# spthm/grace-devel

Measured on AMD Instinct MI355X. Metric: Mrays/s SPH column-density trace, 10^7 particles, higher is better.
Workload: dtype f32

## Files before the change

grace-devel_amd/csrc/trace.hip:

```cpp
#include "kernel_tables.hpp"
#include "trace_kernel.hpp"
#include "trace_plan.hpp"

#include <cmath>

using namespace grace_hip;

namespace grace_hip {

static_assert(GRACE_SPH_KERNEL_TABLE_ROWS == GRACE_SPH_KERNEL_WENDLAND_C6 + 1, "one table per built-in kernel");
__device__ double g_sph_kernel_tables[GRACE_SPH_KERNEL_TABLE_ROWS][N_TABLE] = GRACE_SPH_KERNEL_TABLES_INIT;
static const double k_sph_kernel_tables[GRACE_SPH_KERNEL_TABLE_ROWS][N_TABLE] = GRACE_SPH_KERNEL_TABLES_INIT;

static grace_status trace_state_destroy(Context& c)
{
    if (!c.trace) return GRACE_OK;
    TraceState& ts = *c.trace;
    GRACE_TRY(plan_release(ts));
    GRACE_TRY(scene_release(ts));
    GRACE_TRY(rays_release(ts));
    if (ts.hits.chunk_counts) GRACE_TRY_HIP(hipFree(ts.hits.chunk_counts));
    if (ts.custom_table) GRACE_TRY_HIP(hipFree(ts.custom_table));
    if (ts.status) GRACE_TRY_HIP(hipFree(ts.status));
    if (ts.ev0) GRACE_TRY_HIP(hipEventDestroy(ts.ev0));
// ... 18 lines not shown
    *out = c->trace;
    return GRACE_OK;
}

}

namespace {

struct LaunchPlan {
    int width = 64, n_packets = 0;
    int split = 1;
    bool dev_split = false;
    int hit_chunk_shift = GRANULE_SHIFT, hit_chunks = 0, hit_split = 1;
    size_t hit_packets = 0;
    bool hits_split = false;
    bool keep_chunks = false;
    bool reorder = false;
    bool lattice = false;
    int lat_split = 0;
    bool fast_b = false;
    int treelet = 0, treelet_axis = 0;
};

template <int MODE>
LaunchPlan plan_launch(const TraceState& ts, const bool keep_requested, const size_t n_rays, const size_t n_prims)
{
    LaunchPlan p;
    while ((((n_prims - 1) >> p.hit_chunk_shift) + 1) > size_t(MAX_HIT_CHUNKS)) ++p.hit_chunk_shift;
    p.hit_chunks = int(((n_prims - 1) >> p.hit_chunk_shift) + 1);
    p.hit_packets = ceil_div(n_rays, size_t(64));
    const bool split_hits = ts.width <= 0 && p.hit_packets < 4096 && p.hit_chunks >= 8 && ts.split != 1;
    p.hits_split = MODE == MODE_HITS && split_hits;
    p.keep_chunks = MODE == MODE_COUNT && keep_requested && split_hits;
    if (p.hits_split) {
        if (ts.split > 0) p.hit_split = ts.split;
        else while (p.hit_split < 8 && p.hit_packets * p.hit_split < 16384) p.hit_split *= 2;
    }
    if (ts.width > 0) p.width = ts.width;
    else if (ordered(MODE) && !p.hits_split)
        while (p.width > 16 && ceil_div(n_rays, size_t(p.width)) < 4096) p.width /= 2;
    else if (class_split(MODE) && ts.split <= 0)
        while (p.width > 16 && ceil_div(n_rays, size_t(p.width)) * SUM_CLASSES < 4096) p.width /= 2;
    p.n_packets = ceil_div(n_rays, size_t(p.width));
    p.reorder = ts.ray_reorder && n_rays > 64;
    if (class_split(MODE)) {
        const size_t wave_budget = f4_sums(MODE) ? 16385 : 16384;
        if (ts.split > 0) p.split = ts.split;
        else {
            while (p.split < SUM_CLASSES && size_t(p.n_packets) * p.split < wave_budget) p.split *= 2;
            if (f4_sums(MODE) && p.split > 1 && p.split < ts.lat_split && p.reorder && p.width == 64)
                p.split = ts.lat_split;
        }
    }
    if (p.hits_split) p.split = p.hit_split;
    p.dev_split = f4_class_split(MODE) && p.split > 1 && ts.split <= 0;
    p.lattice = has_lattice(MODE) && p.reorder;
    if (f4_class_split(MODE) && p.split == 1 && p.lattice && p.width == 64
        && ts.lat_split > 0 && ts.split <= 0)
        p.lat_split = ts.lat_split;
    p.fast_b = f4_sums(MODE) && !ts.exact_integrals;
    const int auto_treelet = (MODE == MODE_TRI) ? 512 : 8192, auto_treelet_axis = 32768;
#ifdef GRACE_PACKET_STATS
    p.treelet = ts.treelet < 0 ? auto_treelet : ts.treelet;
    p.treelet_axis = ts.treelet < 0 ? auto_treelet_axis : ts.treelet;
#else
    p.treelet = (MODE == MODE_STATS) ? 0 : (ts.treelet < 0 ? auto_treelet : ts.treelet);
    p.treelet_axis = (MODE == MODE_STATS) ? 0 : (ts.treelet < 0 ? auto_treelet_axis : ts.treelet);
#endif
    return p;
}

struct Nested { bool on = false; size_t* measure = nullptr; };

struct TraceBuffers {
    unsigned long long* sig = nullptr;
    float4* A = nullptr; float2* B = nullptr; double* T64 = nullptr; int2* node_prims = nullptr; float4* C = nullptr;
    float* partial = nullptr; double* partial_d = nullptr;
    int *chunk_counts = nullptr, *chunk_off = nullptr, *scratch_counts = nullptr;
    int4* wave_map = nullptr; int *n_wave_map = nullptr, *pk_first = nullptr, *pk_parts = nullptr;
    uint32_t *pk_prefix = nullptr, *pk_total = nullptr;
    uint32_t* ext = nullptr; uint32_t* keys = nullptr; uint32_t* perm = nullptr;
    bool plan_eligible = false;
    PlanKey plan_key;
};

template <int MODE>
grace_status use_records(TraceState& ts, TraceArgs& a, TraceBuffers& b, FrameGuard& frame, const LaunchPlan& p,
                         const size_t n_rays, const size_t n_prims, const size_t n_nodes, hipStream_t stream,
                         const Nested nested = Nested())
{
    enum CacheUse { USE_NONE, USE_FILL, USE_CHECK, USE_TRUST };
    auto decide = [&](const bool have, const bool pinned, const bool repeat) {
        if (have) return ts.cache_validation ? USE_CHECK : USE_TRUST;
        return (ts.cache_auto && repeat && !pinned) ? USE_FILL : USE_NONE;
    };
    CacheUse scene_use = USE_NONE, rays_use = USE_NONE;
    const SceneKey skey{primitive(MODE), a.spheres, a.nodes, a.leaves, n_prims, n_nodes};
    if (!fp64(MODE) && MODE != MODE_STATS && !nested.measure) {
        scene_use = decide(ts.scene.valid && ts.scene.key == skey, ts.scene.valid && ts.scene.pinned,
                           ts.scene.seen == skey);
        ts.scene.seen = skey;
        if (scene_use == USE_FILL && scene_cache_alloc(ts, skey) != GRACE_OK) scene_use = USE_NONE;
    }
    const RayKey rkey{a.rays, n_rays};
    if (p.reorder && !nested.on) {
        rays_use = decide(ts.rays.valid && ts.rays.key == rkey, ts.rays.valid && ts.rays.pinned,
                          ts.rays.seen == rkey);
        ts.rays.seen = rkey;
        if (rays_use == USE_FILL && rays_cache_alloc(ts, rkey) != GRACE_OK) rays_use = USE_NONE;
    }
    const bool scene_cached = scene_use != USE_NONE, rays_cached = rays_use != USE_NONE;
    auto held = [](const CacheUse u) { return u == USE_CHECK || u == USE_TRUST; };
    b.plan_eligible = ts.plan_on && f4_sums(MODE) && held(scene_use) && held(rays_use) && p.lat_split == 0;
    if (b.plan_eligible)
        b.plan_key = PlanKey{ PLAN_FORMAT, p.fast_b, group_shift(n_prims), p.width, p.reorder, n_rays, n_prims, ts.scene.gen, ts.rays.gen };
    PlanGate gate;
    const bool plan_steady = b.plan_eligible && ts.plan.valid && ts.plan.key == b.plan_key;
    if (plan_steady) {
        gate.ctl = ts.plan.ctl; gate.scene = ts.scene.ctl; gate.rays = ts.rays.ctl;
    }
    const bool scene_sig = scene_use == USE_FILL || scene_use == USE_CHECK;
    const bool rays_sig = rays_use == USE_FILL || rays_use == USE_CHECK, sig = scene_sig || rays_sig;
    auto carve = [&](char* const base) {
        size_t used = 0;
        auto take = [&](auto*& ptr, const size_t count) {
            using T = std::remove_reference_t<decltype(*ptr)>;
            ptr = base ? reinterpret_cast<T*>(base + used) : nullptr;
            used += Workspace::aligned(count * sizeof(T));
        };
        if (sig) take(b.sig, sig_partial_words());
        if (!scene_cached) {
            take(b.A, n_prims + 4);
            if (f4_integrals(MODE)) take(b.B, n_prims + 4);
            if (MODE == MODE_TRI) take(b.T64, 9 * (n_prims + 4));
            take(b.node_prims, n_nodes); take(b.C, cluster_record_count(n_prims));
        }
        if (f4_sums(MODE)) take(b.partial, n_rays * SUM_CLASSES * channels(MODE));
        if (double_sums(MODE)) take(b.partial_d, n_rays * SUM_CLASSES);
        if (p.hits_split) {
            take(b.chunk_counts, n_rays * size_t(p.hit_chunks)); take(b.chunk_off, n_rays * size_t(p.hit_chunks));
            take(b.scratch_counts, n_rays); take(b.wave_map, p.hit_packets * p.hit_split); take(b.n_wave_map, 16);
            take(b.pk_prefix, p.hit_packets * size_t(p.hit_chunks));
            take(b.pk_total, p.hit_packets + 16); take(b.pk_first, p.hit_packets + 16); take(b.pk_parts, p.hit_packets + 16);
        }
        if (p.reorder) { take(b.ext, 20); take(b.keys, n_rays); take(b.perm, n_rays); }
        return used;
    };
    const size_t own = carve(nullptr);
    const size_t need = own + (p.reorder ? sort_ws_bytes(n_rays, 4, 0) : 0);
    if (nested.measure) {
        *nested.measure = need + Workspace::aligned(sig_partial_words() * sizeof(*b.sig));
        return GRACE_OK;
    }
    if (nested.on) GRACE_REQUIRE(Workspace::room() >= need, "trace: the caller's frame is too small for a nested trace");
    else GRACE_TRY(frame.begin(need, stream));
    carve(Workspace::take<char>(own));
    if (sig) {
        SigRequest rq;
        if (scene_sig) {
            rq.prims = a.spheres; rq.prims_bytes = n_prims * (MODE == MODE_TRI ? 36 : 16);
            rq.nodes = a.nodes; rq.nodes_bytes = n_nodes * 64;
            rq.leaves = a.leaves; rq.leaves_bytes = (n_nodes + 1) * 16;
            rq.scene_ctl = ts.scene.ctl; rq.scene_force = scene_use == USE_FILL;
        }
        if (rays_sig) {
            rq.rays = a.rays; rq.rays_bytes = n_rays * 28;
            rq.rays_ctl = ts.rays.ctl; rq.rays_force = rays_use == USE_FILL; rq.rays_ext = ts.rays.ext;
        }
        GRACE_TRY(launch_signatures(rq, b.sig, stream));
    }
    if (scene_cached) {
        Scene& sc = ts.scene;
        if (scene_use != USE_TRUST) {
            GRACE_TRY(scene_fill(skey.kind, a.spheres, n_prims, a.nodes, n_nodes, a.leaves, sc.A, sc.B1, sc.B50,
                                 sc.T64, sc.node_prims, sc.C, stream, &sc.ctl->stale));
            sc.valid = true;
        }
        a.A = sc.A; a.T64 = sc.T64; a.node_prims = sc.node_prims; a.C = sc.C;
        a.B = f4_integrals(MODE) ? (p.fast_b ? sc.B50 : sc.B1) : nullptr;
    } else {
        GRACE_TRY(scene_fill(skey.kind, primitive(MODE) == PRIM_D4 ? static_cast<const void*>(a.spheres_d) : a.spheres,
                             n_prims, a.nodes, n_nodes, a.leaves, b.A, p.fast_b ? nullptr : b.B, p.fast_b ? b.B : nullptr,
                             b.T64, b.node_prims, b.C, stream));
        a.A = b.A; a.B = b.B; a.T64 = b.T64; a.node_prims = b.node_prims; a.C = b.C;
    }
    if (p.reorder) {
        const float4* scene_min = a.C + 2 * ((n_prims + 63) / 64);
        uint32_t* lat_flag = p.lattice ? b.ext + 13 : nullptr;
        int* split_dev = p.dev_split ? reinterpret_cast<int*>(b.ext + 12) : nullptr;
        const int split_flags = f4_sums(MODE) ? SPLIT_WIDE_BUDGET : 0;
        if (rays_cached) {
            RayOrder& ro = ts.rays;
            if (rays_use != USE_TRUST) {
                GRACE_TRY(ray_order(a.rays, n_rays, ro.ext, b.keys, ro.perm, nullptr, nullptr, 0, 0, nullptr,
                                    stream, &ro.ctl->stale));
                ro.valid = true;
            }
            int* plan_split_dev = b.plan_eligible && split_dev && !weighted(MODE)
                ? reinterpret_cast<int*>(b.ext + 16) : nullptr;
            if (lat_flag || split_dev || plan_steady)
                GRACE_TRY(launch_choose_variants(ro.ext, int(n_rays), scene_min, lat_flag, p.n_packets,
                                                 p.split | split_flags, split_dev, stream, plan_steady ? &gate : nullptr,
                                                 plan_split_dev));
            a.perm = ro.perm; a.plan_split_dev = plan_split_dev;
        } else {
            GRACE_TRY(ray_order(a.rays, n_rays, b.ext, b.keys, b.perm, scene_min, lat_flag, p.n_packets,
                                p.split | split_flags, split_dev, stream));
            a.perm = b.perm;
        }
        a.lat_dev = reinterpret_cast<const int*>(lat_flag); a.split_dev = split_dev;
    }
    return GRACE_OK;
}

template <int MODE, bool SPLIT, bool ALT = false>
void launch_walk(const int grid, const TraceArgs& args, hipStream_t stream)
{
    trace_kernel<MODE, SPLIT, ALT, false><<<grid, TRACE_BLOCK, 0, stream>>>(args);
    if constexpr (has_lattice(MODE))
        if (args.lat_dev) trace_kernel<MODE, SPLIT, ALT, true><<<grid, TRACE_BLOCK, 0, stream>>>(args);
}

template <int MODE>
grace_status dispatch(const TraceState& ts, const TraceArgs& a, const TraceBuffers& b, const LaunchPlan& p,
                      const int* kept, const size_t n_rays, hipStream_t stream)
{
    const int grid = ceil_div(size_t(p.n_packets) * p.split, TRACE_BLOCK / 64);
    const int* const plan_k_dev = a.plan_usable ? a.plan_split_dev : nullptr;
    auto combine = [&](const int k, const int* k_dev, const int* run_if) -> grace_status {
        const int g = ceil_div(n_rays * channels(MODE), 256);
        if constexpr (double_sums(MODE))
            combine_classes_kernel<double><<<g, 256, 0, stream>>>(a.partial_d, int(n_rays), k, k_dev, a.out_sums_d, run_if);
        else if constexpr (weighted(MODE))
            combine_channel_classes_kernel<<<g, 256, 0, stream>>>(a.partial, int(n_rays), channels(MODE), k, k_dev,
                                                                  a.out_sums, a.out_stride, run_if,
                                                                  a.plan_usable, plan_k_dev);
        else if constexpr (f4_sums(MODE))
            combine_classes_kernel<float><<<g, 256, 0, stream>>>(a.partial, int(n_rays), k, k_dev, a.out_sums, run_if,
                                                                 a.plan_usable, plan_k_dev);
        else return GRACE_OK;
        GRACE_CHECK_LAUNCH();
        return GRACE_OK;
    };
    if constexpr (class_split(MODE)) {
        auto walk = [&](auto alt_tag) -> grace_status {
            constexpr bool ALT = decltype(alt_tag)::value;
            if constexpr (has_lattice(MODE)) if (p.lat_split) {
                if (output(MODE) == OUT_COUNTS)
                    GRACE_TRY_HIP(hipMemsetAsync(a.out_counts, 0, n_rays * sizeof(int), stream));
                trace_kernel<MODE, false, ALT, false><<<grid, TRACE_BLOCK, 0, stream>>>(a);
                GRACE_CHECK_LAUNCH();
                TraceArgs a_lat = a;
                a_lat.split = p.lat_split; a_lat.split_dev = nullptr;
                trace_kernel<MODE, true, ALT, true><<<ceil_div(size_t(p.n_packets) * p.lat_split, TRACE_BLOCK / 64),
                                                      TRACE_BLOCK, 0, stream>>>(a_lat);
                GRACE_CHECK_LAUNCH();
                return combine(p.lat_split, nullptr, a.lat_dev);
            }
            if constexpr (f4_sums(MODE)) if (a.plan_usable) {
                GRACE_TRY(plan_record(ts, a, stream));
                const int grid_planned = a.plan_split_dev
                    ? ceil_div(size_t(p.n_packets) * planned_split(p.n_packets), TRACE_BLOCK / 64) : grid;
                GRACE_TRY(launch_planned(MODE, ALT, grid_planned, a, stream));
                if (p.split == 1) GRACE_TRY(combine(1, nullptr, reinterpret_cast<const int*>(a.plan_usable)));
            }
            if (p.split > 1) launch_walk<MODE, true, ALT>(grid, a, stream);
            else launch_walk<MODE, false, ALT>(grid, a, stream);
            return GRACE_OK;
        };
        if constexpr (f4_sums(MODE)) GRACE_TRY(p.fast_b ? walk(std::true_type()) : walk(std::false_type()));
        else GRACE_TRY(walk(std::false_type()));
    } else if constexpr (MODE == MODE_HITS) {
        if (p.hits_split) {
            const int* counts = kept;
            if (!kept) {
                TraceArgs c = a;
                c.chunk_counts = b.chunk_counts; c.out_counts = b.scratch_counts;
                GRACE_TRY_HIP(hipMemsetAsync(b.chunk_counts, 0, n_rays * size_t(p.hit_chunks) * 4, stream));
                GRACE_TRY_HIP(hipMemsetAsync(b.scratch_counts, 0, n_rays * 4, stream));
                launch_walk<MODE_COUNT, true>(grid, c, stream);
                GRACE_CHECK_LAUNCH();
                counts = b.chunk_counts;
            }
            hits_offsets_kernel<<<ceil_div(n_rays, 4), 256, 0, stream>>>(counts, a.offsets, int(n_rays),
                                                                         p.hit_chunks, b.chunk_off);
            GRACE_CHECK_LAUNCH();
            hits_plan_kernel<<<p.n_packets, MAX_HIT_CHUNKS, 0, stream>>>(counts, a.perm, int(n_rays),
                                                                         p.hit_chunks, b.pk_prefix, b.pk_total);
            GRACE_CHECK_LAUNCH();
            hits_assign_kernel<<<1, 1024, 0, stream>>>(b.pk_total, p.n_packets, p.n_packets * p.split, p.hit_chunks,
                                                       b.pk_first, b.pk_parts, b.n_wave_map,
                                                       ts.hits_stage_split ? 200000ull : 0ull);
            GRACE_CHECK_LAUNCH();
            hits_bounds_kernel<<<p.n_packets, 64, 0, stream>>>(b.pk_prefix, b.pk_total, b.pk_first, b.pk_parts,
                                                               p.hit_chunks, b.wave_map);
            GRACE_CHECK_LAUNCH();
            TraceArgs staged = a, direct = a;
            staged.stage_dev = direct.stage_dev = b.n_wave_map + 4;
            staged.stage_want = 1; direct.stage_want = 0;
            launch_walk<MODE, true, true>(grid, staged, stream);
            GRACE_CHECK_LAUNCH();
            launch_walk<MODE, true, false>(grid, direct, stream);
        } else if (p.n_packets >= 4096) {
            launch_walk<MODE, false, true>(grid, a, stream);
        } else {
            launch_walk<MODE, false, false>(grid, a, stream);
        }
    } else {
        launch_walk<MODE, false>(grid, a, stream);
    }
    GRACE_CHECK_LAUNCH();
    GRACE_TRY(stamps_report(MODE));
    if (p.split > 1) GRACE_TRY(combine(p.split, a.split_dev, nullptr));
    return GRACE_OK;
}

template <int MODE>
grace_status launch_trace(TraceArgs a, size_t n_rays, size_t n_spheres, size_t n_nodes,
                          hipStream_t stream, const Nested nested = Nested())
{
    GRACE_REQUIRE(a.rays && a.spheres && a.nodes && a.leaves && a.root, "trace: null pointer");
    GRACE_REQUIRE(n_rays < (size_t(1) << 31), "trace: bad ray count");
    GRACE_REQUIRE(n_nodes >= 1 && n_nodes < (size_t(1) << 30), "trace: bad node count");
    GRACE_REQUIRE(n_spheres > 0 && n_spheres < (size_t(1) << 31), "trace: bad primitive count");
    TraceState* ts_ptr = nullptr;
    GRACE_TRY(trace_state(&ts_ptr));
    TraceState& ts = *ts_ptr;
    GRACE_TRY(ensure_status(ts, stream));
    a.kernel_table = ts.kernel_table;
    const LaunchPlan p = plan_launch<MODE>(ts, a.keep_chunks, n_rays, n_spheres);
    const bool reuse_chunks = p.hits_split && ts.hits.valid && ts.hits.rays == a.rays
        && ts.hits.n_rays == n_rays && ts.hits.prims == static_cast<const void*>(a.spheres)
        && ts.hits.n_prims == n_spheres && ts.hits.n_chunks == p.hit_chunks;
    if (chunked(MODE)) ts.hits.valid = false;
    const size_t need = n_rays * size_t(p.hit_chunks);
    if (p.keep_chunks && ts.hits.capacity < need) {
        if (ts.hits.chunk_counts) { GRACE_TRY_HIP(hipDeviceSynchronize()); GRACE_TRY_HIP(hipFree(ts.hits.chunk_counts)); }
        ts.hits.chunk_counts = nullptr; ts.hits.capacity = 0;
        hipError_t e = hipMalloc(reinterpret_cast<void**>(&ts.hits.chunk_counts), need * sizeof(int));
        if (e != hipSuccess) return set_error(GRACE_OUT_OF_MEMORY, __FILE__, __LINE__, hipGetErrorString(e));
        ts.hits.capacity = need;
    }
    FrameGuard frame;
    TraceBuffers b;
    GRACE_TRY(use_records<MODE>(ts, a, b, frame, p, n_rays, n_spheres, n_nodes, stream, nested));
    if (nested.measure) return GRACE_OK;
    a.width = p.width; a.split = p.split; a.treelet = p.treelet; a.treelet_axis = p.treelet_axis;
    a.n_rays = int(n_rays); a.n_nodes = int(n_nodes); a.n_prims = int(n_spheres); a.status = ts.status;
    a.group_shift = group_shift(n_spheres); a.chunk_shift = p.hit_chunk_shift; a.n_chunks = p.hit_chunks;
    a.partial = b.partial; a.partial_d = b.partial_d;
    a.chunk_off = b.chunk_off; a.wave_map = b.wave_map; a.n_wave_map = b.n_wave_map;
    if (p.split > 1 && output(MODE) == OUT_COUNTS)
        GRACE_TRY_HIP(hipMemsetAsync(a.out_counts, 0, n_rays * sizeof(int), stream));
    if (p.keep_chunks && p.split > 1) {
        a.chunk_counts = ts.hits.chunk_counts;
        GRACE_TRY_HIP(hipMemsetAsync(ts.hits.chunk_counts, 0, n_rays * size_t(p.hit_chunks) * 4, stream));
        ts.hits.valid = true; ts.hits.rays = a.rays; ts.hits.n_rays = n_rays;
        ts.hits.prims = a.spheres; ts.hits.n_prims = n_spheres; ts.hits.n_chunks = p.hit_chunks;
    }
    ts.last_lat_dev = a.lat_dev; ts.last_lat_stream = stream;
    if constexpr (f4_sums(MODE)) {
        PacketPlan& pp = ts.plan;
        if (b.plan_eligible && !(pp.key == b.plan_key && (pp.valid || pp.dead)))
            GRACE_TRY(plan_fill(ts, b.plan_key, a, stream));
        ts.last_plan_ctl = nullptr;
        if (b.plan_eligible && pp.valid && pp.key == b.plan_key) {
            a.plan_idx = pp.idx; a.plan_hdr = pp.hdr; a.plan_spans = pp.spans; a.plan_counts = pp.counts;
            a.plan_usable = &pp.ctl->usable;
            ts.last_plan_ctl = pp.ctl; ts.last_plan_stream = stream;
            ts.last_plan_fuses = !weighted(MODE) && p.fast_b;
        }
    }
    return timed(ts, stream, [&] {
        return dispatch<MODE>(ts, a, b, p, reuse_chunks ? ts.hits.chunk_counts : nullptr, n_rays, stream);
    });
}

TraceArgs trace_args(const void* d_rays, const void* d_prims, const int* d_nodes, const int* d_leaves,
                     const int* d_root)
{
    TraceArgs a = {};
    a.rays = static_cast<const float*>(d_rays);
    a.spheres = static_cast<const float4*>(d_prims);
    a.nodes = reinterpret_cast<const float4*>(d_nodes);
    a.leaves = reinterpret_cast<const int4*>(d_leaves);
    a.root = d_root;
    return a;
}

}

namespace grace_hip {
grace_status rays_invalidate_if_written(const void* d_written)
{
    Context* c = nullptr;
    GRACE_TRY(current_context(&c));
    if (!c->trace) return GRACE_OK;
    TraceState& ts = *c->trace;
    if (ts.cache_validation) return GRACE_OK;
    if (ts.rays.valid && d_written && d_written == static_cast<const void*>(ts.rays.key.rays)) return rays_release(ts);
    return GRACE_OK;
}

grace_status scene_invalidate_if_written(const void* d_written)
{
    Context* c = nullptr;
    GRACE_TRY(current_context(&c));
    if (!c->trace) return GRACE_OK;
    TraceState& ts = *c->trace;
    if (ts.cache_validation) return GRACE_OK;
    if (ts.scene.valid && d_written
        && (d_written == ts.scene.key.prims || d_written == ts.scene.key.nodes || d_written == ts.scene.key.leaves))
        return scene_release(ts);
    return GRACE_OK;
}

grace_status trace_nested_bytes(size_t n_rays, size_t n_spheres, size_t n_nodes, size_t* bytes)
{
    TraceArgs a = trace_args(bytes, bytes, reinterpret_cast<const int*>(bytes), reinterpret_cast<const int*>(bytes),
                             reinterpret_cast<const int*>(bytes));
    size_t counts = 0, hits = 0;
    GRACE_TRY(launch_trace<MODE_COUNT>(a, n_rays, n_spheres, n_nodes, nullptr, Nested{true, &counts}));
    GRACE_TRY(launch_trace<MODE_HITS>(a, n_rays, n_spheres, n_nodes, nullptr, Nested{true, &hits}));
    *bytes = counts > hits ? counts : hits;
    return GRACE_OK;
}

grace_status trace_hitcounts_nested(const void* d_rays, size_t n_rays, const float* d_spheres, size_t n_spheres,
                                    const int* d_nodes, size_t n_nodes, const int* d_leaves, const int* d_root,
                                    int* d_hit_counts, hipStream_t stream)
{
    TraceArgs a = trace_args(d_rays, d_spheres, d_nodes, d_leaves, d_root);
    a.out_counts = d_hit_counts;
    return launch_trace<MODE_COUNT>(a, n_rays, n_spheres, n_nodes, stream, Nested{true, nullptr});
}

grace_status trace_hits_nested(const void* d_rays, size_t n_rays, const float* d_spheres, size_t n_spheres,
                               const int* d_nodes, size_t n_nodes, const int* d_leaves, const int* d_root,
                               const int* d_ray_offsets, int* d_hit_indices, float* d_hit_integrals,
                               float* d_hit_distances, hipStream_t stream)
{
    TraceArgs a = trace_args(d_rays, d_spheres, d_nodes, d_leaves, d_root);
    a.offsets = d_ray_offsets;
    a.hit_idx = d_hit_indices;
    a.hit_integral = d_hit_integrals;
    a.hit_dist = d_hit_distances;
    return launch_trace<MODE_HITS>(a, n_rays, n_spheres, n_nodes, stream, Nested{true, nullptr});
// ... 276 lines not shown
    GRACE_TRACE_STATE();
    GRACE_REQUIRE(ts.timing && ts.ev_valid, "no timed traversal launch recorded");
    GRACE_TRY_HIP(hipEventSynchronize(ts.ev1));
    GRACE_TRY_HIP(hipEventElapsedTime(h_ms, ts.ev0, ts.ev1));
    return GRACE_OK;
}

grace_status grace_trace_last_lattice(int* h_lattice)
{
    GRACE_REQUIRE(h_lattice, "null output");
    *h_lattice = 0;
    GRACE_TRACE_STATE();
    if (ts.last_lat_dev) {
        GRACE_TRY_HIP(hipStreamSynchronize(ts.last_lat_stream));
        GRACE_TRY_HIP(hipMemcpy(h_lattice, ts.last_lat_dev, sizeof(int), hipMemcpyDeviceToHost));
    }
    return GRACE_OK;
}

grace_status grace_trace_last_plan_used(int* h_used)
{
    GRACE_REQUIRE(h_used, "null output");
    *h_used = 0;
    GRACE_TRACE_STATE();
    if (ts.last_plan_ctl) {
        PlanCtl h = {};
        GRACE_TRY_HIP(hipStreamSynchronize(ts.last_plan_stream));
        GRACE_TRY_HIP(hipMemcpy(&h, ts.last_plan_ctl, sizeof(h), hipMemcpyDeviceToHost));
        *h_used = h.usable != 0u ? 1 : 0;
    }
    return GRACE_OK;
}

grace_status grace_trace_plan_stats(unsigned long long* h_stats)
{
    GRACE_REQUIRE(h_stats, "null output");
    for (int k = 0; k < 7; ++k) h_stats[k] = 0;
    GRACE_TRACE_STATE();
    if (ts.last_plan_ctl) {
        PlanCtl h = {};
        GRACE_TRY_HIP(hipStreamSynchronize(ts.last_plan_stream));
        GRACE_TRY_HIP(hipMemcpy(&h, ts.last_plan_ctl, sizeof(h), hipMemcpyDeviceToHost));
        if (h.usable != 0u) {
            for (int k = 0; k < 6; ++k) h_stats[k] = h.stats[k];
            h_stats[6] = h.largest_round;
        }
    }
    return GRACE_OK;
}

grace_status grace_trace_plan_loops(unsigned long long* h_loops)
{
    GRACE_REQUIRE(h_loops, "null output");
    h_loops[0] = h_loops[1] = 0;
    GRACE_TRACE_STATE();
    if (ts.last_plan_ctl) {
        PlanCtl h = {};
        GRACE_TRY_HIP(hipStreamSynchronize(ts.last_plan_stream));
        GRACE_TRY_HIP(hipMemcpy(&h, ts.last_plan_ctl, sizeof(h), hipMemcpyDeviceToHost));
        if (h.usable != 0u) {
            h_loops[0] = ts.last_plan_fuses ? h.loops : h.stats[2];
            h_loops[1] = ts.last_plan_fuses ? h.largest_loop : h.largest_round;
        }
    }
    return GRACE_OK;
}

grace_status grace_trace_set_plan(int on)
{
    GRACE_TRACE_STATE();
    ts.plan_on = on != 0;
    if (!ts.plan_on) GRACE_TRY(plan_release(ts));
    return GRACE_OK;
}

grace_status grace_trace_set_plan_budget(size_t bytes)
{
    GRACE_TRACE_STATE();
    ts.plan_budget = bytes;
    GRACE_TRY(plan_release(ts));
    return GRACE_OK;
}

grace_status grace_trace_plan_bytes(size_t* h_bytes)
{
    GRACE_REQUIRE(h_bytes, "null output");
    GRACE_TRACE_STATE();
    const PacketPlan& pp = ts.plan;
    *h_bytes = pp.valid ? pp.bytes() : 0;
    return GRACE_OK;
}

grace_status grace_trace_set_packet_split(int waves_per_packet)
{
    GRACE_REQUIRE(waves_per_packet == -1 || waves_per_packet == 1 || waves_per_packet == 2
                      || waves_per_packet == 4 || waves_per_packet == 8,
                  "packet split must be 1, 2, 4, 8 or -1 (automatic)");
    GRACE_TRACE_STATE();
    ts.split = waves_per_packet;
    return GRACE_OK;
}

grace_status grace_trace_set_packet_width(int rays_per_packet)
{
    GRACE_REQUIRE(rays_per_packet == -1 || rays_per_packet == 16 || rays_per_packet == 32
                      || rays_per_packet == 64,
                  "packet width must be 16, 32, 64 or -1 (automatic)");
    GRACE_TRACE_STATE();
    ts.width = rays_per_packet;
    return GRACE_OK;
}

grace_status grace_trace_set_exact_integrals(int enabled)
{
    GRACE_TRACE_STATE();
    ts.exact_integrals = enabled != 0;
    return GRACE_OK;
}

grace_status grace_trace_set_sph_kernel(int kind)
{
    GRACE_REQUIRE(kind >= GRACE_SPH_KERNEL_CUBIC && kind <= GRACE_SPH_KERNEL_WENDLAND_C6,
                  "set_sph_kernel: kind must be a built-in GRACE_SPH_KERNEL_* (0..5); a custom table is "
                  "set with grace_trace_set_sph_kernel_table");
    GRACE_TRACE_STATE();
    ts.sph_kernel = kind;
    ts.kernel_table = ts.builtin_tables + kind * N_TABLE;
    return GRACE_OK;
}

grace_status grace_trace_set_sph_kernel_table(const double* h_table, int n)
{
    GRACE_REQUIRE(h_table && n == N_TABLE, "set_sph_kernel_table: the table must hold 51 values");
    for (int i = 0; i < N_TABLE; ++i)
        GRACE_REQUIRE(std::isfinite(h_table[i]) && h_table[i] >= 0.0,
                      "set_sph_kernel_table: every value must be finite and >= 0");
    GRACE_REQUIRE(h_table[N_TABLE - 1] == 0.0, "set_sph_kernel_table: the last value (b = H) must be 0");
    GRACE_TRACE_STATE();
    GRACE_TRY_HIP(hipDeviceSynchronize());
    if (!ts.custom_table)
        GRACE_TRY_HIP(hipMalloc(reinterpret_cast<void**>(&ts.custom_table), N_TABLE * sizeof(double)));
    GRACE_TRY_HIP(hipMemcpy(ts.custom_table, h_table, N_TABLE * sizeof(double), hipMemcpyHostToDevice));
    for (int i = 0; i < N_TABLE; ++i) ts.custom_host[i] = h_table[i];
    ts.sph_kernel = GRACE_SPH_KERNEL_CUSTOM;
    ts.kernel_table = ts.custom_table;
    return GRACE_OK;
}

grace_status grace_trace_get_sph_kernel(int* h_kind, double* h_table51)
{
    GRACE_TRACE_STATE();
    if (h_kind) *h_kind = ts.sph_kernel;
    if (h_table51) {
        const double* t = ts.sph_kernel == GRACE_SPH_KERNEL_CUSTOM ? ts.custom_host
                                                                   : k_sph_kernel_tables[ts.sph_kernel];
        for (int i = 0; i < N_TABLE; ++i) h_table51[i] = t[i];
    }
    return GRACE_OK;
}

grace_status grace_trace_set_treelet_size(int max_primitives)
{
    GRACE_REQUIRE(max_primitives >= -1, "treelet size must be >= 0 (or -1 for automatic)");
    GRACE_TRACE_STATE();
    ts.treelet = max_primitives;
    return GRACE_OK;
// ... 68 lines not shown
```

grace-devel_amd/csrc/trace_coherence.hip:

```cpp
#include "trace_state.hpp"

using namespace grace_hip;

namespace {

__device__ __forceinline__ uint32_t f2ord_u(float f)
{
    const uint32_t u = __float_as_uint(f);
    return (u & 0x80000000u) ? ~u : (u | 0x80000000u);
}

__device__ __forceinline__ float ord2f_u(uint32_t u)
{
    return __uint_as_float((u & 0x80000000u) ? (u & 0x7fffffffu) : ~u);
}

__global__ void ray_ext_init_kernel(uint32_t* __restrict__ ext16)
{
    if (threadIdx.x < 16) ext16[threadIdx.x] = threadIdx.x < 6 ? 0xFFFFFFFFu : 0u;
}

__global__ __launch_bounds__(1024) void ray_extents_kernel(const float* __restrict__ rays, int n,
                                                          uint32_t* __restrict__ ext12,
                                                          const uint32_t* __restrict__ run_if)
// ... 85 lines not shown
    int dims[2] = { 0, 0 }, nvar = 0;
    float lo[2] = { 0.f, 0.f }, span[2] = { 0.f, 0.f };
    for (int k = 5; k >= 0; --k) {
        const float l = ord2f_u(ext12[k]), sp = ord2f_u(ext12[6 + k]) - l;
        if (sp > 0.f && sp < INFINITY) {
            if (nvar < 2) { dims[nvar] = k; lo[nvar] = l; span[nvar] = sp; }
            ++nvar;
        }
    }
    bool fit = nvar == 2 && n >= 64 && (n & (n - 1)) == 0;
    float m1 = 0.f, m2 = 0.f;
    if (fit) {
        int log_n = 0;
        while ((1 << log_n) < n) ++log_n;
        fit = false;
        const float ratio = span[0] / span[1];
        for (int a = 3; a <= log_n - 3; ++a) {
            const float c1 = float((1 << a) - 1), c2 = float((1 << (log_n - a)) - 1);
            if (fabsf(c1 / c2 - ratio) <= 1e-3f * ratio) { fit = true; m1 = c1; m2 = c2; break; }
        }
    }
    if (!fit) {
        if (blockIdx.x == 0 && threadIdx.x == 0) atomicOr(flag, 1u);
        return;
    }
    const float s1 = m1 / span[0], s2 = m2 / span[1];
    bool off = false;
    for (int i = blockIdx.x * blockDim.x + threadIdx.x; i < n; i += gridDim.x * blockDim.x) {
        const float* r = rays + 7 * size_t(i);
        const float u1 = (r[dims[0]] - lo[0]) * s1, u2 = (r[dims[1]] - lo[1]) * s2;
        off = off || !(fabsf(u1 - rintf(u1)) <= 0.01f) || !(fabsf(u2 - rintf(u2)) <= 0.01f);
    }
    if (__builtin_amdgcn_ballot_w64(off) != 0ull && (threadIdx.x & 63) == 0) atomicOr(flag, 1u);
}

__device__ void choose_variants(const uint32_t* __restrict__ ext12, int n, const float4* __restrict__ scene_min,
                                uint32_t* __restrict__ lat_flag, int split_packets, int split_launched,
                                int* __restrict__ split_dev)
{
    if (lat_flag) {
        int n_dir = 0;
        bool one_dir = true;
        float e1 = 0.f, e2 = 0.f;
        for (int k = 0; k < 3; ++k) {
            const float dl = ord2f_u(ext12[k]), dh = ord2f_u(ext12[6 + k]);
            one_dir = one_dir && dl == dh;
            n_dir += dl != 0.f ? 1 : 0;
            const float e = ord2f_u(ext12[9 + k]) - ord2f_u(ext12[3 + k]);
            if (e > e1) { e2 = e1; e1 = e; } else if (e > e2) e2 = e;
        }
        const float spacing2 = e1 * e2 / float(n);
        const float r2_min = scene_min->x;
        bool lat = one_dir && n_dir == 1 && spacing2 > 0.f && r2_min < 2.0f * spacing2;
        if (!lat && e1 == 0.f && ext12[15] != 0u) {
            const float len = ord2f_u(ext12[15]);
            if (len > 0.f && len < INFINITY) lat = r2_min < 2.0f * (12.566371f * len * len / float(n));
        }
        *lat_flag = lat ? 1u : 0u;
    }
    if (split_dev)
        *split_dev = choose_split(ext12, split_packets, split_launched, lat_flag ? *lat_flag != 0u : false);
}

__global__ void choose_variants_kernel(const uint32_t* __restrict__ ext12, int n, const float4* __restrict__ scene_min,
                                       uint32_t* __restrict__ lat_flag, int split_packets, int split_launched,
                                       int* __restrict__ split_dev, const PlanGate gate,
                                       int* __restrict__ plan_split_dev)
{
    if (lat_flag || split_dev)
        choose_variants(ext12, n, scene_min, lat_flag, split_packets, split_launched, split_dev);
    if (plan_split_dev) *plan_split_dev = planned_split(split_packets);
    if (gate.ctl) {
        PlanCtl& pc = *gate.ctl;
        const bool stale = pc.sig[0] != gate.scene->sig[0] || pc.sig[1] != gate.scene->sig[1]
            || pc.sig[2] != gate.rays->sig[0] || pc.sig[3] != gate.rays->sig[1];
        pc.record = stale ? 1u : 0u;
        if (stale) {
            pc.unusable = 0u; pc.usable = 1u;
            pc.sig[0] = gate.scene->sig[0]; pc.sig[1] = gate.scene->sig[1];
            pc.sig[2] = gate.rays->sig[0]; pc.sig[3] = gate.rays->sig[1];
            for (int k = 0; k < 6; ++k) pc.stats[k] = 0ull;
            pc.largest_round = 0u;
            pc.loops = 0ull; pc.largest_loop = 0u;
        }
    }
}

__global__ __launch_bounds__(256) void ray_keys_kernel(const float* __restrict__ rays, int n,
                                                       const uint32_t* __restrict__ ext12,
                                                       uint32_t* __restrict__ keys,
                                                       const float4* __restrict__ scene_min,
                                                       uint32_t* __restrict__ lat_flag,
                                                       int split_packets, int split_launched,
                                                       int* __restrict__ split_dev,
                                                       const uint32_t* __restrict__ not_grid,
                                                       const uint32_t* __restrict__ run_if)
{
    if (run_if && *run_if == 0u) return;
    const bool z_order_2d = not_grid && *not_grid == 0u;
    if (blockIdx.x == 0 && threadIdx.x == 0)
        choose_variants(ext12, n, scene_min, lat_flag, split_packets, split_launched, split_dev);
    float lo[6], scale[6], span[6];
    int nvar = 0;
    float span_d = 0.f, span_o = 0.f;
#pragma unroll
    for (int k = 0; k < 6; ++k) {
        lo[k] = ord2f_u(ext12[k]);
        span[k] = ord2f_u(ext12[6 + k]) - lo[k];
        const bool varies = span[k] > 0.f && span[k] < INFINITY;
        if (varies) { if (k < 3) span_d = fmaxf(span_d, span[k]); else span_o = fmaxf(span_o, span[k]); }
    }
#pragma unroll
    for (int k = 0; k < 6; ++k) {
        const bool varies = span[k] > 0.f && span[k] < INFINITY;
        scale[k] = varies ? 1.0f / (k < 3 ? span_d : span_o) : 0.f;
        nvar += varies ? 1 : 0;
    }
    const int bits = nvar ? min(15, 30 / nvar) : 0;
    const float qmax = float((1 << bits) - 1);
    const bool pencil = scale[3] == 0.f && scale[4] == 0.f && scale[5] == 0.f && nvar > 0;
    for (int i = blockIdx.x * blockDim.x + threadIdx.x; i < n; i += gridDim.x * blockDim.x) {
        const float* r = rays + 7 * size_t(i);
        if (pencil) {
            const float l1 = fabsf(r[0]) + fabsf(r[1]) + fabsf(r[2]);
            float u = r[0] / l1, v = r[1] / l1;
            if (r[2] < 0.f) {
                const float fu = (1.f - fabsf(v)) * (u >= 0.f ? 1.f : -1.f);
                const float fv = (1.f - fabsf(u)) * (v >= 0.f ? 1.f : -1.f);
                u = fu; v = fv;
            }
            const uint32_t qu = uint32_t(fminf(32767.f, fmaxf(0.f, (u * 0.5f + 0.5f) * 32767.f + 0.5f)));
            const uint32_t qv = uint32_t(fminf(32767.f, fmaxf(0.f, (v * 0.5f + 0.5f) * 32767.f + 0.5f)));
            keys[i] = hilbert2d_15(qu, qv);
            continue;
        }
        uint32_t q[6];
#pragma unroll
        for (int k = 0; k < 6; ++k) q[k] = uint32_t(fminf(qmax, (r[k] - lo[k]) * scale[k] * qmax + 0.5f));
#ifndef GRACE_MORTON2D
        if (nvar == 2 && !z_order_2d) {
            uint32_t xy[2] = {0, 0};
            int m = 0;
#pragma unroll
            for (int k = 5; k >= 0; --k)
                if (scale[k] > 0.f) { if (m < 2) xy[m] = q[k]; ++m; }
            keys[i] = hilbert2d_15(xy[1], xy[0]);
            continue;
        }
#endif
        uint32_t key = 0;
        for (int b = bits - 1; b >= 0; --b) {
#pragma unroll
            for (int k = 5; k >= 0; --k)
                if (scale[k] > 0.f) key = (key << 1) | ((q[k] >> b) & 1u);
        }
        keys[i] = key << (30 - bits * nvar);
    }
}

}

namespace grace_hip {

grace_status launch_choose_variants(const uint32_t* ext12, int n, const float4* scene_min, uint32_t* lat_flag,
                                    int split_packets, int split_launched, int* split_dev, hipStream_t stream,
                                    const PlanGate* gate, int* plan_split_dev)
// ... 101 lines not shown
```

grace-devel_amd/csrc/trace_kernel.hpp:

```cpp
#pragma once

#include "trace_diag.hpp"
#include "trace_packet.hpp"
#include "trace_state.hpp"

#include <type_traits>

namespace {

using namespace grace_hip;

__device__ __forceinline__ bool any_lane(bool p) { return __builtin_amdgcn_ballot_w64(p) != 0ull; }

__device__ __forceinline__ int imin(int a, int b) { return a < b ? a : b; }
__device__ __forceinline__ int imax(int a, int b) { return a > b ? a : b; }

__device__ __forceinline__ void aabbs_hit(const float ix, const float iy, const float iz,
                                          const float ox, const float oy, const float oz,
                                          const float len, const float4 L, const float4 R,
                                          const float4 Z, bool& hit_l, bool& hit_r)
{
    const float bx_L = (L.x - ox) * ix, tx_L = (L.y - ox) * ix;
    const float by_L = (L.z - oy) * iy, ty_L = (L.w - oy) * iy;
    const float bz_L = (Z.x - oz) * iz, tz_L = (Z.y - oz) * iz;
// ... 130 lines not shown
__device__ __forceinline__ bool pencil_may_hit(const float4 s, const Pencil& pc)
{
    const float vx = s.x - pc.ox, vy = s.y - pc.oy, vz = s.z - pc.oz;
    const float d2 = __builtin_fmaf(vx, vx, __builtin_fmaf(vy, vy, vz * vz));
    const float va = __builtin_fmaf(vx, pc.ax, __builtin_fmaf(vy, pc.ay, vz * pc.az));
    const float inv = __builtin_amdgcn_rsqf(d2);
    const float sin_a = fminf(1.0f, __builtin_amdgcn_sqrtf(s.w) * inv * 1.00001f);
    const float cos_a = __builtin_amdgcn_sqrtf(fmaxf(0.0f, __builtin_fmaf(-sin_a, sin_a, 1.0f)));
    const float cos_limit = __builtin_fmaf(pc.cos_t, cos_a, -pc.sin_t * sin_a) - 1e-5f;
    const float h = __builtin_amdgcn_sqrtf(s.w) * 1.00001f + 1e-6f * __builtin_amdgcn_sqrtf(d2);
    float out = -1.0f;
#pragma unroll
    for (int k = 0; k < 4; ++k)
        out = fmaxf(out, __builtin_fmaf(vx, pc.nx[k], __builtin_fmaf(vy, pc.ny[k], vz * pc.nz[k])) - h);
    return !(d2 > s.w * 1.00001f) || (!(va * inv < cos_limit) && !(out > 0.0f));
}

template <int AX, bool FUSED = false>
__device__ __forceinline__ bool axis_beam_may_hit(const float4 s, const Beam& bm)
{
    constexpr int D1 = AX == 0 ? 1 : 0, D2 = AX == 2 ? 1 : 2;
    const float s1 = AX == 0 ? s.y : s.x;
    const float s2 = AX == 2 ? s.y : s.z;
    const float q1 = s1 - __builtin_amdgcn_fmed3f(s1, bm.olo[D1], bm.ohi[D1]);
    const float q2 = s2 - __builtin_amdgcn_fmed3f(s2, bm.olo[D2], bm.ohi[D2]);
    const float b2_lo = FUSED ? __builtin_fmaf(q1, q1, q2 * q2) : q1 * q1 + q2 * q2;
    return !(b2_lo >= s.w);
}

__device__ __forceinline__ float4 cluster_sphere(const float4 blo, const float4 bhi)
{
    const float cx = 0.5f * (blo.x + bhi.x), cy = 0.5f * (blo.y + bhi.y), cz = 0.5f * (blo.z + bhi.z);
    const float ex = bhi.x - cx, ey = bhi.y - cy, ez = bhi.z - cz;
    const float fx = cx - blo.x, fy = cy - blo.y, fz = cz - blo.z;
    const float rx = fmaxf(ex, fx), ry = fmaxf(ey, fy), rz = fmaxf(ez, fz);
    return make_float4(cx, cy, cz, (rx * rx + ry * ry + rz * rz) * 1.001f);
}

template <int AX>
__device__ __forceinline__ bool cluster_may_hit(const float4 blo, const float4 bhi, const Beam& bm,
                                                const Pencil* pc)
{
    if constexpr (AX >= 0) {
        constexpr int D1 = AX == 0 ? 1 : 0, D2 = AX == 2 ? 1 : 2;
        const float lo1 = AX == 0 ? blo.y : blo.x, hi1 = AX == 0 ? bhi.y : bhi.x;
        const float lo2 = AX == 2 ? blo.y : blo.z, hi2 = AX == 2 ? bhi.y : bhi.z;
        return !(lo1 > bm.ohi[D1]) && !(hi1 < bm.olo[D1]) && !(lo2 > bm.ohi[D2]) && !(hi2 < bm.olo[D2]);
    } else if constexpr (AX == -2) {
        const float lx = blo.x - pc->ox, ly = blo.y - pc->oy, lz = blo.z - pc->oz;
        const float hx = bhi.x - pc->ox, hy = bhi.y - pc->oy, hz = bhi.z - pc->oz;
        const float scale = fmaxf(fmaxf(fmaxf(fabsf(lx), fabsf(hx)), fmaxf(fabsf(ly), fabsf(hy))),
                                  fmaxf(fabsf(lz), fabsf(hz)));
        const float slack = 1e-5f * scale;
        float worst = -1.0f;
#pragma unroll
        for (int k = 0; k < 4; ++k) {
            const float m = fminf(pc->nx[k] * lx, pc->nx[k] * hx) + fminf(pc->ny[k] * ly, pc->ny[k] * hy)
                + fminf(pc->nz[k] * lz, pc->nz[k] * hz);
            worst = fmaxf(worst, m);
        }
        const float front = fmaxf(pc->ax * lx, pc->ax * hx) + fmaxf(pc->ay * ly, pc->ay * hy)
            + fmaxf(pc->az * lz, pc->az * hz);
        return !(worst > slack) && !(front < -slack) && pencil_may_hit(cluster_sphere(blo, bhi), *pc);
    } else {
        return beam_may_hit(cluster_sphere(blo, bhi), bm, 1.52587890625e-05f );
    }
}

typedef int plan_i32x4 __attribute__((ext_vector_type(4)));
typedef uint32_t plan_u32x4 __attribute__((ext_vector_type(4), aligned(4)));
template <typename T>
__device__ __forceinline__ const __attribute__((address_space(4))) T* plan_const(const void* p)
{
    return (const __attribute__((address_space(4))) T*)(uintptr_t)p;
}

template <int N>
struct WeightedB {
    float x, y;
    float w[N + 1];
    __device__ WeightedB(const float2 b) : x(b.x), y(b.y), w{} {}
};

template <int MODE, bool SPLIT, bool ALT = false, bool LAT = false, bool PLANNED = false>
__global__ __launch_bounds__(TRACE_BLOCK, !f4_class_split(MODE) ? 1
                                          : weighted(MODE) ? (channels(MODE) == 1 ? 6 : 7 - channels(MODE))
                                          : (SPLIT ? 8 : 6))
void trace_kernel(const TraceArgs a)
{
    static_assert(!ALT || f4_integrals(MODE), "no alternative path for this mode");
    static_assert(!LAT || has_lattice(MODE), "no lattice cull for this mode");
    static_assert(!PLANNED || (SPLIT && !LAT && f4_sums(MODE)), "planned: class-split column densities only");
    if constexpr (PLANNED) {
        if (*plan_const<uint32_t>(a.plan_usable) == 0u) return;
    } else if (has_lattice(MODE)) {
        if (a.plan_usable && *a.plan_usable != 0u) return;
        if (a.lat_dev ? (*a.lat_dev != 0) != LAT : LAT) return;
        if (a.stage_dev && *a.stage_dev != a.stage_want) return;
    }
    constexpr bool FAST = ALT && f4_sums(MODE);
    constexpr bool WEIGHTED = weighted(MODE);
    constexpr int NW = channels(MODE), WP = WEIGHTED ? (NW + 1) / 2 : 0;
    using BRec = std::conditional_t<WEIGHTED, WeightedB<NW>, float2>;
    constexpr bool FUSE = PLANNED && !WEIGHTED && FAST;
    __shared__ double2 s_lut[FAST ? 1 : N_TABLE];
    constexpr int LUTF_N = 256;
    __shared__ float2 s_lutf[FAST ? LUTF_N : 1];
    constexpr bool D4 = primitive(MODE) == PRIM_D4, F4D = primitive(MODE) == PRIM_F4D;
    constexpr bool LDS_TILE = primitive(MODE) == PRIM_F4;
    __shared__ __align__(16) float2 s_tile[LDS_TILE ? TRACE_BLOCK / 64 : 1][LDS_TILE ? (FUSE ? 4 : 3 + WP) : 1][LDS_TILE ? 66 : 1];
    static_assert(!FUSE || 4 * 66 * sizeof(float2) >= (PLAN_LOOP_MAX + 2) * sizeof(float4), "the fused loop's tile");
    __shared__ double s_tile_d[D4 ? TRACE_BLOCK / 64 : 1][D4 ? 64 : 1][D4 ? 6 : 1];
    __shared__ float4 s_tile_f[F4D ? TRACE_BLOCK / 64 : 1][F4D ? 64 : 1][F4D ? 2 : 1];
    const int lane = threadIdx.x & 63;
    static_assert(!SPLIT || class_split(MODE) || MODE == MODE_HITS, "triangle and stats walks do not split");
    constexpr bool RANGE_SPLIT = SPLIT && MODE == MODE_HITS;
    const int split_ordinary = !SPLIT ? 1 : (!RANGE_SPLIT && a.split_dev) ? *a.split_dev : a.split;
    int split_planned = 0;
    if constexpr (PLANNED)
        if (a.plan_split_dev) split_planned = *plan_const<int>(a.plan_split_dev);
    const int split = PLANNED && split_planned > 0 ? split_planned : split_ordinary;
    const int n_packets = (a.n_rays + a.width - 1) / a.width;
    const int nb = (n_packets * split + TRACE_BLOCK / 64 - 1) / (TRACE_BLOCK / 64);
    const int q = nb >> 3, r8 = nb & 7, xcd = blockIdx.x & 7, slot = blockIdx.x >> 3;
    if (slot >= q + (xcd < r8 ? 1 : 0)) return;
    const int vblock = (xcd < r8 ? xcd * (q + 1) : r8 * (q + 1) + (xcd - r8) * q) + slot;
    const int wave_id = __builtin_amdgcn_readfirstlane(vblock * (TRACE_BLOCK / 64)
                                                       + (threadIdx.x >> 6));
    if (integrates(MODE)) {
        if (FAST) {
            static_assert(TRACE_BLOCK >= 256, "one table entry per thread");
            float2 e = make_float2(0.f, 0.f);
            if (threadIdx.x < N_TABLE - 1) {
                const double y0 = a.kernel_table[threadIdx.x], dy = a.kernel_table[threadIdx.x + 1] - y0;
                e = make_float2(float(y0 - double(threadIdx.x) * dy), float(dy));
            }
            if (threadIdx.x < LUTF_N) s_lutf[threadIdx.x] = e;
        } else if (threadIdx.x < N_TABLE) {
            const int i0 = threadIdx.x;
            const double y0 = a.kernel_table[i0];
            const double y1 = i0 + 1 < N_TABLE ? a.kernel_table[i0 + 1] : y0;
            s_lut[threadIdx.x] = make_double2(y0, y1 - y0);
        }
        __syncthreads();
    }
    int packet = wave_id / split, part = wave_id - packet * split;
    int prim_lo = 0, prim_hi = 0x7fffffff;
    if (RANGE_SPLIT) {
        if (wave_id >= *a.n_wave_map) return;
        const int4 wm = a.wave_map[wave_id];
        packet = wm.x; part = 0;
        prim_lo = wm.y << a.chunk_shift;
        prim_hi = wm.z << a.chunk_shift;
        if (prim_lo >= prim_hi) return;
    }
    const int first_ray = packet * a.width;
    if (first_ray >= a.n_rays) return;
    const int classes_per_part = SUM_CLASSES / split;
    const int own_lo = part * classes_per_part, own_hi = own_lo + classes_per_part;
    auto owns_granule = [&](const int g) {
        if (RANGE_SPLIT) { const int p = g << GRANULE_SHIFT; return p >= prim_lo && p < prim_hi; }
        const int c = g & (SUM_CLASSES - 1);
        return c >= own_lo && c < own_hi;
    };
    auto foreign_range = [&](const int first, const int count) {
        if (RANGE_SPLIT) return first + count <= prim_lo || first >= prim_hi;
        const int g0 = first >> GRANULE_SHIFT, g1 = (first + count - 1) >> GRANULE_SHIFT;
        return g1 - g0 <= 1 && !owns_granule(g0) && !owns_granule(g1);
    };
    const PacketRay ray = load_packet_ray(a, first_ray, lane);
    const bool valid = ray.valid;
    const int ray_index = ray.index;
    const float dx = ray.dx, dy = ray.dy, dz = ray.dz;
    const float ox = ray.ox, oy = ray.oy, oz = ray.oz;
    const float len = ray.len;
    const float ix = 1.f / dx, iy = 1.f / dy, iz = 1.f / dz;
    const Beam beam = packet_beam(ray);
    int axis = -1;
    if (!ordered(MODE)) axis = packet_axis(dx, dy, dz);
    __shared__ Pencil s_pencil[TRACE_BLOCK / 64];
    Pencil pencil;
    bool is_pencil = false;
    if (!PLANNED && axis < 0 && MODE != MODE_STATS && beam.olo[0] == beam.ohi[0] && beam.olo[1] == beam.ohi[1]
        && beam.olo[2] == beam.ohi[2]) {
        float sx = dx, sy = dy, sz = dz;
#pragma unroll
        for (int off = 32; off > 0; off >>= 1) {
            sx += __shfl_xor(sx, off); sy += __shfl_xor(sy, off); sz += __shfl_xor(sz, off);
        }
        const float inv = 1.0f / sqrtf(sx * sx + sy * sy + sz * sz);
        const float ax = sx * inv, ay = sy * inv, az = sz * inv;
        const float cx = ay * dz - az * dy, cy = az * dx - ax * dz, cz = ax * dy - ay * dx;
        const float sin_t = wave_max(sqrtf(cx * cx + cy * cy + cz * cz)) + 2e-6f;
        const float cos_min = wave_min(ax * dx + ay * dy + az * dz);
// ... 366 lines not shown
                m4 = a.A[pj];
                if (LDS_TILE && NEED_B) m2 = a.B[pj];
                if (D4) mined_next = reinterpret_cast<const double4*>(a.spheres_d)[pj];
                if (F4D) {
                    const float4 f = a.spheres[pj];
                    mined_next = make_double4(f.x, f.y, f.z, f.w);
                }
                if constexpr (WEIGHTED) {
#pragma unroll
                    for (int c = 0; c < NW; ++c) mw_next[c] = a.weights[size_t(pj) * a.w_stride + c];
                }
            };
            for (int cg = c_first; cg <= (PLANNED ? c_first : c_last); cg += 64) {
                const unsigned long long st_t1 = STAMP_NOW(); (void)st_t1;
                unsigned long long cmask = 1ull;
                unsigned long long small_mask = ~0ull;
                if (!PLANNED && c_last != c_first) {
                    const int cj = min(cg + lane, c_last);
                    const float4 blo = a.C[2 * size_t(cj)], bhi = a.C[2 * size_t(cj) + 1];
                    const bool c_may = cluster_may_hit<AX>(blo, bhi, beam, &s_pencil[wv]);
                    if (LATTICE && AX >= 0) small_mask = __builtin_amdgcn_ballot_w64(blo.w < s_lat_r2[wv]);
                    const int n_c = min(64, c_last - cg + 1);
                    cmask = __builtin_amdgcn_ballot_w64(c_may)
                        & (n_c >= 64 ? ~0ull : ((1ull << n_c) - 1ull));
                    if (SPLIT) cmask &= __builtin_amdgcn_ballot_w64(owns_granule(cj >> (GRANULE_SHIFT - 6)));
#ifdef GRACE_PACKET_STATS
                    if (MODE == MODE_STATS) st_leaves += 1;
#endif
                }
                STAMP_ADD(st_cluster, st_t1);
                if (cmask == 0ull) continue;
                int cnext = cg + __builtin_ctzll(cmask);
                cmask &= cmask - 1ull;
                plan_u32x4 plan_h = { 0u, 0u, 0u, 0u };
                uint32_t plan_word = 0u, plan_word2 = 0u;
                int plan_i = 0, plan_w = 0, loop_n = 0, loop_bits = 0;
                (void)plan_h; (void)plan_word; (void)plan_word2; (void)plan_i; (void)plan_w; (void)loop_n; (void)loop_bits;
                const uint32_t lane4 = uint32_t(lane) << 2;
                (void)lane4;
                auto headers_at = [&](const int round) {
                    return *reinterpret_cast<const __attribute__((address_space(4))) plan_u32x4*>(plan_hdr_at + round);
                };
                (void)headers_at;
                auto form_loop = [&]() {
                    if constexpr (PLANNED) {
                        loop_n = 0;
                        if (plan_i < plan_n) {
                            loop_n = plan_header_count(plan_h.x);
                            loop_bits = plan_header_bits(plan_h.x);
                            ++plan_i;
                            if constexpr (FUSE) {
                                int k = 1;
                                for (;;) {
                                    if (k == 4) { plan_h = headers_at(plan_i); k = 0; }
                                    const uint32_t next = k == 0 ? plan_h.x : k == 1 ? plan_h.y : k == 2 ? plan_h.z : plan_h.w;
                                    if (!(plan_i < plan_n && planned_fuses(loop_n, loop_bits, next))) break;
                                    loop_n += plan_header_count(next);
                                    ++plan_i; ++k;
                                }
                            }
                        }
                        plan_h = headers_at(plan_i);
                        const char* const base = reinterpret_cast<const char*>(plan_idx_at + plan_w);
                        plan_word = *reinterpret_cast<const uint32_t*>(base + lane4);
                        if constexpr (FUSE)
                            if (loop_n > 64) plan_word2 = *reinterpret_cast<const uint32_t*>(base + 256 + lane4);
                    }
                };
                if constexpr (PLANNED) {
                    plan_h = headers_at(0);
                    form_loop();
                }
                float4 mine_next;
                float2 mineb_next = make_float2(0.f, 0.f);
                int round_n_next = 0;
                uint32_t round_bits_next = 0u;
                float4 mine2_next = make_float4(0.f, 0.f, 0.f, 0.f);
                float2 mine2b_next = make_float2(0.f, 0.f);
                (void)round_n_next; (void)round_bits_next; (void)mine2_next; (void)mine2b_next;
                auto gather_round = [&]() {
                    if constexpr (PLANNED) {
                        round_n_next = loop_n;
                        round_bits_next = uint32_t(loop_bits);
                        const int pj = int(min(plan_word, uint32_t(r_hi - 1)));
                        mine_next = a.A[pj];
                        if (NEED_B) mineb_next = a.B[pj];
                        if constexpr (WEIGHTED) {
#pragma unroll
                            for (int c = 0; c < NW; ++c) mw_next[c] = a.weights[size_t(pj) * a.w_stride + c];
                        }
                        if constexpr (FUSE) {
                            if (loop_n > 64) {
                                const int pj2 = int(min(plan_word2, uint32_t(r_hi - 1)));
                                mine2_next = a.A[pj2];
                                mine2b_next = a.B[pj2];
                            }
                        }
                        plan_w += loop_n;
                        form_loop();
                    }
                };
                if constexpr (PLANNED) gather_round();
                else load_cluster(cnext, mine_next, mineb_next);
                for (;;) {
                    const unsigned long long st_t2 = STAMP_NOW(); (void)st_t2;
                    const int pbase = cnext << 6;
                    const float4 mine = mine_next;
                    const float2 mineb = mineb_next;
                    const double4 mined = mined_next;
                    float mw[NW];
                    if constexpr (WEIGHTED) {
#pragma unroll
                        for (int c = 0; c < NW; ++c) mw[c] = mw_next[c];
                    }
                    bool more = cmask != 0ull;
                    const int round_n = round_n_next;
                    const uint32_t round_bits = round_bits_next;
                    (void)round_n; (void)round_bits;
                    const float4 mine2 = mine2_next;
                    const float2 mine2b = mine2b_next;
                    (void)mine2; (void)mine2b;
                    if constexpr (PLANNED) {
                        more = loop_n > 0;
                        if (more) gather_round();
                    } else if (more) {
                        cnext = cg + __builtin_ctzll(cmask);
                        cmask &= cmask - 1ull;
                        load_cluster(cnext, mine_next, mineb_next);
                    }
                    const int lo_bit = max(r_lo - pbase, 0), hi_bit = min(r_hi - pbase, 64);
                    const unsigned long long m_mask =
                        (hi_bit >= 64 ? ~0ull : ((1ull << hi_bit) - 1ull)) & (~0ull << lo_bit);
                bool may_hit = false;
                if constexpr (PLANNED) { }
                else if constexpr (AX >= 0) may_hit = axis_beam_may_hit<AX, FAST>(mine, beam);
                else if constexpr (AX == -2) may_hit = pencil_may_hit(mine, s_pencil[wv]);
                else may_hit = beam_may_hit(mine, beam);
                unsigned long long rest = PLANNED
                    ? (round_n >= 64 ? ~0ull : ((1ull << round_n) - 1ull))
                    : (__builtin_amdgcn_ballot_w64(may_hit) & m_mask);
                bool keep = __builtin_amdgcn_inverse_ballot_w64(rest);
                bool lean_round = PLANNED && (__builtin_amdgcn_readfirstlane(int(round_bits)) & 1) != 0;
                if constexpr (!PLANNED && AX >= 0 && f4_class_split(MODE)) {
                    const float sa = AX == 0 ? mine.x : AX == 1 ? mine.y : mine.z;
                    const unsigned long long inside =
                        __builtin_amdgcn_ballot_w64(__builtin_fmaf(sa, da0, noda_lo) >= 0.0f)
                        & __builtin_amdgcn_ballot_w64(__builtin_fmaf(sa, da0, noda_hi) < len_lo);
                    lean_round = same_sense & ((rest & ~inside) == 0ull);
                }
                bool fat_round = PLANNED && (__builtin_amdgcn_readfirstlane(int(round_bits)) & 2) != 0;
                if constexpr (LEAN4 && !PLANNED)
                    fat_round = (rest & ~__builtin_amdgcn_ballot_w64(mine.w >= fat_r2)) == 0ull;
                if constexpr (LATTICE && AX >= 0) {
                    if (((small_mask >> ((pbase >> 6) - cg)) & 1ull) && rest != 0ull
                        && __builtin_amdgcn_ballot_w64(keep && mine.w < s_lat_r2[wv]) != 0ull) {
                        const float s1 = AX == 0 ? mine.y : mine.x;
                        const float s2 = AX == 2 ? mine.y : mine.z;
                        float q1 = INFINITY, q2 = INFINITY;
#pragma unroll 1
                        for (int k = 0; k < 8; ++k) {
                            q1 = fminf(q1, fabsf(s1 - s_lat[wv][0][k]));
                            q2 = fminf(q2, fabsf(s2 - s_lat[wv][1][k]));
                        }
                        const float nan_if_nan = (s1 + s2) * 0.0f;
                        const float b2_lo = (FAST ? __builtin_fmaf(q1, q1, q2 * q2) : q1 * q1 + q2 * q2) + nan_if_nan;
                        keep = keep && !(b2_lo >= mine.w);
                        rest = __builtin_amdgcn_ballot_w64(keep);
                    }
                }
#ifdef GRACE_PACKET_STATS
                if (MODE == MODE_STATS) { st_tested += __builtin_popcountll(rest); }
#endif
                constexpr bool COMPACT = f4_class_split(MODE);
                bool skip_round = rest == 0ull;
                if (!PLANNED && !skip_round && (CLASSES || SPLIT)) {
                    const int pf = pbase + __builtin_ctzll(rest);
// ... 137 lines not shown
                            a.hit_dist_d[write_at] = dot_p;
                            ++write_at;
                        }
                    } else if (MODE == MODE_TRI) {
                        float t;
                        if (tri_intersect(ddx, ddy, ddz, ox, oy, oz, a.T64 + 9 * size_t(jj), &t)) {
                            if (t <= tri_tmin && t >= 1E-14f) {
                                tri_tmin = t;
                                tri_data = jj;
                            }
                        }
                    } else {
                        float b2, dot_p;
                        if (AX >= 0) {
                            const float sa = AX == 0 ? s.x : AX == 1 ? s.y : s.z;
                            const float s1 = AX == 0 ? s.y : s.x;
                            const float s2 = AX == 2 ? s.y : s.z;
                            const float q1 = s1 - o1, q2 = s2 - o2;
                            dot_p = LEAN ? 0.0f : __builtin_fmaf(sa, da, noda);
                            b2 = FAST ? __builtin_fmaf(q1, q1, q2 * q2) : q1 * q1 + q2 * q2;
                        } else {
                            const float px = s.x - ox, py = s.y - oy, pz = s.z - oz;
                            dot_p = px * dx + py * dy + pz * dz;
                            const float bx = px - dot_p * dx;
                            const float by = py - dot_p * dy;
                            const float bz = pz - dot_p * dz;
                            b2 = FAST ? __builtin_fmaf(bx, bx, __builtin_fmaf(by, by, bz * bz))
                                      : bx * bx + by * by + bz * bz;
                        }
                        if constexpr (FAST && LEAN) {
                            const float b = fminf(__builtin_amdgcn_sqrtf(b2) * sb.x, float(N_TABLE - 1));
                            const float2 y = s_lutf[static_cast<int>(b)];
                            if constexpr (WEIGHTED) {
                                const float t = __builtin_fmaf(y.y, b, y.x);
#pragma unroll
                                for (int c = 0; c < NW; ++c) wsum[c] = __builtin_fmaf(t, sb.w[c], wsum[c]);
                            } else {
                                sum = __builtin_fmaf(__builtin_fmaf(y.y, b, y.x), sb.y, sum);
                            }
                            return;
                        }
                        const bool hit = LEAN ? !(b2 >= s.w)
                                              : !(b2 >= s.w) && !(dot_p < 0.0f) && !(dot_p >= len);
#ifdef GRACE_PACKET_STATS
                        if (MODE == MODE_STATS && __builtin_amdgcn_ballot_w64(hit) != 0ull) ++st_nodes;
#endif
                        if (!integrates(MODE)) {
                            count += hit ? 1 : 0;
                        } else if (hit) {
                            const float w = FAST ? hit_integral_fast(b2, sb.x, s_lutf)
                                                 : hit_integral(b2, sb.x, sb.y, s_lut);
                            if constexpr (WEIGHTED) {
#pragma unroll
                                for (int c = 0; c < NW; ++c)
                                    wsum[c] = FAST ? __builtin_fmaf(w, sb.w[c], wsum[c]) : wsum[c] + sb.w[c] * w;
                            } else {
                            if (FAST) {
                                sum = __builtin_fmaf(w, sb.y, sum);
                            } else if (MODE == MODE_CUMULATIVE) {
                                sum += w;
                            } else if (valid && !STAGE_HITS) {
                                a.hit_idx[write_at] = jj;
                                a.hit_integral[write_at] = w;
                                a.hit_dist[write_at] = dot_p;
                                ++write_at;
                            } else if (valid) {
                                const int wvh = threadIdx.x >> 6;
                                s_hits[wvh][0][staged][lane] = __int_as_float(jj);
                                s_hits[wvh][STAGE_HITS ? 1 : 0][staged][lane] = w;
                                s_hits[wvh][STAGE_HITS ? 2 : 0][staged][lane] = dot_p;
                                ++staged;
                                ++write_at;
                            }
                            }
                        }
                        if (STAGE_HITS && __builtin_amdgcn_ballot_w64(staged == HIT_CAP) != 0ull)
                            drain_hits();
                    }
                };
                auto fetch = [&](unsigned long long& td, int& k, float4& c, BRec& cb, int& jj) {
                    int at;
                    if (COMPACT) {
                        at = k++;
                        jj = 0;
                    } else {
                        at = __builtin_ctzll(td);
                        td = (td & ~(1ull << at)) | 0x8000000000000000ull;
                        jj = min(pbase + at, r_hi - 1);
                    }
                    if (LDS_TILE) {
                        const float2 xy = s_tile[wv][0][at];
                        const float2 zw = s_tile[wv][LDS_TILE ? 1 : 0][at];
                        c = make_float4(xy.x, xy.y, zw.x, zw.y);
                        if constexpr (WEIGHTED) {
                            const float2 b = s_tile[wv][2][at];
                            cb.x = b.x; cb.y = b.y;
#pragma unroll
                            for (int p = 0; p < WP; ++p) {
                                const float2 wp = s_tile[wv][3 + p][at];
                                cb.w[2 * p] = wp.x;
                                cb.w[2 * p + 1] = wp.y;
                            }
                        } else {
                        if (NEED_B) cb = s_tile[wv][LDS_TILE ? 2 : 0][at];
                        }
                        __builtin_amdgcn_sched_barrier(0);
                    } else if (!fp64(MODE)) {
                        c = a.A[jj];
                    }
                };
                auto run = [&](auto lean_tag) {
                    float4 c0, c1, c2;
                    BRec b0 = make_float2(0.f, 0.f), b1 = b0, b2 = b0;
                    int j0, j1 = 0, j2 = 0;
                    int left = __builtin_popcountll(todo);
                    unsigned long long td = todo | 0x8000000000000000ull;
                    int k = 0;
                    fetch(td, k, c0, b0, j0);
                    fetch(td, k, c1, b1, j1);
                    for (;;) {
                        fetch(td, k, c2, b2, j2);
                        process(lean_tag, c0, b0, j0);
                        if (--left == 0) break;
                        fetch(td, k, c0, b0, j0);
                        process(lean_tag, c1, b1, j1);
                        if (--left == 0) break;
                        fetch(td, k, c1, b1, j1);
                        process(lean_tag, c2, b2, j2);
                        if (--left == 0) break;
                    }
                };
                auto run_lean4 = [&](auto fat_tag) {
                    constexpr bool FAT = decltype(fat_tag)::value;
                    float4 c0, c1, c2;
                    int left = FUSE ? round_n : __builtin_popcountll(todo);
                    const float4* t4 = tile4;
                    if constexpr (WEIGHTED && NW > 1) {
                        float4 x0, x1;
                        auto procw = [&](const float4 c, const float4 x) {
                            const float q1 = c.x - o1, q2 = c.y - o2;
                            float b = __builtin_amdgcn_sqrtf(__builtin_fmaf(q1, q1, q2 * q2)) * c.z;
                            if (!FAT) b = fminf(b, float(N_TABLE - 1));
                            const float2 y = s_lutf[static_cast<int>(b)];
                            const float t = __builtin_fmaf(y.y, b, y.x);
                            const float xw[4] = { c.w, x.x, x.y, x.z };
#pragma unroll
                            for (int ch = 0; ch < NW; ++ch) wsum[ch] = __builtin_fmaf(t, xw[ch], wsum[ch]);
                        };
                        c0 = t4[0]; x0 = t4[66]; __builtin_amdgcn_sched_barrier(0);
                        for (;;) {
                            c1 = t4[1]; x1 = t4[67]; __builtin_amdgcn_sched_barrier(0);
                            procw(c0, x0);
                            if (--left == 0) break;
                            c0 = t4[2]; x0 = t4[68]; __builtin_amdgcn_sched_barrier(0);
                            procw(c1, x1);
                            if (--left == 0) break;
                            t4 += 2;
                        }
                        return;
                    }
                    auto proc = [&](const float4 c) {
                        const float q1 = c.x - o1, q2 = c.y - o2;
                        float b = __builtin_amdgcn_sqrtf(__builtin_fmaf(q1, q1, q2 * q2)) * c.z;
                        if (!FAT) b = fminf(b, float(N_TABLE - 1));
                        const float2 y = s_lutf[static_cast<int>(b)];
                        if constexpr (WEIGHTED) wsum[0] = __builtin_fmaf(__builtin_fmaf(y.y, b, y.x), c.w, wsum[0]);
                        else sum = __builtin_fmaf(__builtin_fmaf(y.y, b, y.x), c.w, sum);
                    };
                    c0 = t4[0]; __builtin_amdgcn_sched_barrier(0);
                    c1 = t4[1]; __builtin_amdgcn_sched_barrier(0);
                    for (;;) {
                        c2 = t4[2]; __builtin_amdgcn_sched_barrier(0);
                        proc(c0);
                        if (--left == 0) break;
                        c0 = t4[3]; __builtin_amdgcn_sched_barrier(0);
                        proc(c1);
                        if (--left == 0) break;
                        c1 = t4[4]; __builtin_amdgcn_sched_barrier(0);
                        proc(c2);
                        if (--left == 0) break;
                        t4 += 3;
                    }
                };
                if constexpr (LEAN4) {
                    if (lean_round) {
                        if (fat_round) run_lean4(std::true_type());
                        else run_lean4(std::false_type());
                    } else run(std::false_type());
                } else {
                    if (lean_round) run(std::true_type());
                    else run(std::false_type());
                }
                STAMP_ADD(st_surv, st_t3);
                }
                    if (!more) break;
                }
            }
            };
            switch (axis) {
            case 0: sweep_range(std::integral_constant<int, 0>()); break;
            case 1: sweep_range(std::integral_constant<int, 1>()); break;
            case 2: sweep_range(std::integral_constant<int, 2>()); break;
            default:
                if constexpr (!PLANNED) {
                    if (is_pencil) sweep_range(std::integral_constant<int, -2>());
                    else sweep_range(std::integral_constant<int, -1>());
                }
                break;
            }
            junk |= warm;
        }
    }

#ifdef GRACE_STAMPS
    if (lane == 0) {
        atomicAdd(&g_stamp_acc[0], __builtin_amdgcn_s_memtime() - st_begin);
        atomicAdd(&g_stamp_acc[1], st_walk); atomicAdd(&g_stamp_acc[2], st_cluster);
        atomicAdd(&g_stamp_acc[3], st_cull); atomicAdd(&g_stamp_acc[4], st_surv);
        atomicAdd(&g_stamp_acc[5], st_rounds); atomicAdd(&g_stamp_acc[6], st_nsurv);
        atomicAdd(&g_stamp_acc[7], 1ull);
        {
            const unsigned slot = atomicAdd(&g_stamp_n, 1u) & 0xffffu;
            g_stamp_log[slot][0] = st_begin; g_stamp_log[slot][1] = __builtin_amdgcn_s_memtime();
            g_stamp_log[slot][2] = st_nsurv; g_stamp_log[slot][3] = st_walk;
        }
    }
#endif
    if (STAGE_HITS) drain_hits();
    if (CHUNKED && MODE == MODE_COUNT && a.chunk_counts) leave_chunk();
    if ((overflow || junk < 0) && lane == 0) *a.status = GRACE_STACK_OVERFLOW;
    if (!valid) return;
    if (output(MODE) == OUT_COUNTS) {
        if (!SPLIT) a.out_counts[ray_index] = count;
        else if (count) atomicAdd(&a.out_counts[ray_index], count);
    }
    if (MODE == MODE_TRI) a.out_counts[ray_index] = tri_data;
    if (double_sums(MODE)) {
        if (cur_granule >= 0) s_class_d[wv_acc][cur_granule & (SUM_CLASSES - 1)][lane] = sum_d;
        const int c_lo = SPLIT ? own_lo : 0, c_n = SPLIT ? classes_per_part : SUM_CLASSES;
        for (int w = 1; w < c_n; w *= 2)
            for (int c = c_lo; c < c_lo + c_n; c += 2 * w) {
                const double x = s_class_d[wv_acc][c][lane], y = s_class_d[wv_acc][c + w][lane];
                s_class_d[wv_acc][c][lane] = x + y;
            }
        if (!SPLIT) a.out_sums_d[ray_index] = s_class_d[wv_acc][0][lane];
        else a.partial_d[size_t(ray_index) * split + part] = s_class_d[wv_acc][c_lo][lane];
    }
    if (MODE == MODE_CUMULATIVE) {
        if (cur_granule >= 0) s_class[wv_acc][cur_granule & (SUM_CLASSES - 1)][lane] = sum;
        float t[SUM_CLASSES];
#pragma unroll
        for (int c = 0; c < SUM_CLASSES; ++c) t[c] = s_class[wv_acc][c][lane];
        float result = 0.f;
        if (!SPLIT) {
#pragma unroll
            for (int w = 1; w < SUM_CLASSES; w *= 2)
#pragma unroll
                for (int c = 0; c < SUM_CLASSES; c += 2 * w) t[c] = t[c] + t[c + w];
            result = t[0];
            a.out_sums[ray_index] = result;
        } else {
            for (int w = 1; w < classes_per_part; w *= 2)
                for (int c = own_lo; c < own_hi; c += 2 * w) {
                    const float x = s_class[wv_acc][c][lane], y = s_class[wv_acc][c + w][lane];
// ... 39 lines not shown
```

grace-devel_amd/csrc/trace_planned.hip:

```cpp
#include "trace_kernel.hpp"

#include <vector>

using namespace grace_hip;

namespace {

struct PlanRef {
    uint32_t* idx;
    uint32_t* hdr;
    const int4* spans;
    int4* counts;
    PlanCtl* ctl;
    int force;
};

template <bool FUSED>
__global__ __launch_bounds__(TRACE_BLOCK) void plan_record_kernel(const TraceArgs a, const PlanRef pl)
{
    __shared__ float s_lat[TRACE_BLOCK / 64][2][8];
    if (pl.spans && !pl.force && pl.ctl->record == 0u) return;
    const int lane = threadIdx.x & 63, wv = threadIdx.x >> 6;
    const int n_packets = (a.n_rays + a.width - 1) / a.width;
    const int packet = blockIdx.x * (TRACE_BLOCK / 64) + wv;
    if (packet >= n_packets) return;
    const PacketRay ray = load_packet_ray(a, packet * a.width, lane);
    const int axis = packet_axis(ray.dx, ray.dy, ray.dz);
    const float4* const group_boxes = a.C + 2 * ((size_t(a.n_prims) + 63) >> 6) + 1;
    const int covered = min(__float_as_int(group_boxes[-1].y), a.n_prims);
    int cnt = 0;
    int round_n = 0, round_bits = 0;
    int t_surv = 0, t_rounds = 0, t_full = 0, t_cap = 0, t_flag = 0, t_max = 0;
    int loop_n = 0, loop_bits = 0, t_loops = 0, t_lmax = 0;
    auto round_closed = [&](const int n, const int bits) {
        if (FUSED && loop_n > 0 && planned_fuses(loop_n, loop_bits, plan_header(n, bits))) {
            loop_n += n;
        } else {
            if (loop_n > 0) { t_loops += 1; t_lmax = max(t_lmax, loop_n); }
            loop_n = n; loop_bits = bits;
        }
    };
    bool failed = axis < 0 || covered < 0;
    if (!failed) {
        const AxisRay ar = axis_ray(axis, ray);
        float noda_lo, noda_hi, len_lo, da0;
        bool same_sense;
        axis_extremes(ar, ray.len, noda_lo, noda_hi, len_lo, da0, same_sense);
        const float lo1 = wave_min(ar.o1), hi1 = wave_max(ar.o1), lo2 = wave_min(ar.o2), hi2 = wave_max(ar.o2);
        const float ea = ar.oa + ar.da * ray.len;
        const float alo = wave_min(fminf(ar.oa, ea)), ahi = wave_max(fmaxf(ar.oa, ea));
        const float fat_r2 = fat_radius2(hi1 - lo1, hi2 - lo2);
        bool lat_ok;
        float cell2;
        build_origin_lattice(ar.o1, ar.o2, lane, s_lat, lat_ok, cell2);
        const float lat_r2 = lat_ok ? cell2 : 0.f;

        auto box_may_hit = [&](const float4 blo, const float4 bhi, const bool along) {
            const float l1 = axis == 0 ? blo.y : blo.x, h1 = axis == 0 ? bhi.y : bhi.x;
            const float l2 = axis == 2 ? blo.y : blo.z, h2 = axis == 2 ? bhi.y : bhi.z;
            const float la = axis == 0 ? blo.x : axis == 1 ? blo.y : blo.z;
            const float ha = axis == 0 ? bhi.x : axis == 1 ? bhi.y : bhi.z;
            return !(l1 > hi1) && !(h1 < lo1) && !(l2 > hi2) && !(h2 < lo2)
                && (!along || (!(la > ahi) && !(ha < alo)));
        };
        const int n_groups = int((size_t(covered) + (size_t(1) << a.group_shift) - 1) >> a.group_shift);
        for (int g0 = 0; g0 < n_groups; g0 += 64) {
            const int gj = min(g0 + lane, n_groups - 1);
            const bool g_may = box_may_hit(group_boxes[2 * size_t(gj)], group_boxes[2 * size_t(gj) + 1], true);
            const int n_g = min(64, n_groups - g0);
            unsigned long long gmask = __builtin_amdgcn_ballot_w64(g_may) & (n_g >= 64 ? ~0ull : ((1ull << n_g) - 1ull));
            while (gmask != 0ull) {
                const int g = g0 + __builtin_ctzll(gmask);
                gmask &= gmask - 1ull;
                const int r_lo = g << a.group_shift;
                const int r_hi = r_lo + min(1 << a.group_shift, covered - r_lo);
                const int c_first = r_lo >> 6, c_last = (r_hi - 1) >> 6;
                for (int cg = c_first; cg <= c_last; cg += 64) {
                    const int cj = min(cg + lane, c_last);
                    const bool c_may = box_may_hit(a.C[2 * size_t(cj)], a.C[2 * size_t(cj) + 1], false);
                    const int n_c = min(64, c_last - cg + 1);
                    unsigned long long cmask = __builtin_amdgcn_ballot_w64(c_may)
                        & (n_c >= 64 ? ~0ull : ((1ull << n_c) - 1ull));
                    while (cmask != 0ull) {
                        const int c = cg + __builtin_ctzll(cmask);
                        cmask &= cmask - 1ull;
                        const int pbase = c << 6;
                        const int pj = min(max(pbase + lane, r_lo), r_hi - 1);
                        const float4 mine = a.A[pj];
                        const int lo_bit = max(r_lo - pbase, 0), hi_bit = min(r_hi - pbase, 64);
                        const unsigned long long m_mask =
                            (hi_bit >= 64 ? ~0ull : ((1ull << hi_bit) - 1ull)) & (~0ull << lo_bit);
                        const float s1 = axis == 0 ? mine.y : mine.x;
                        const float s2 = axis == 2 ? mine.y : mine.z;
                        const float sa = axis == 0 ? mine.x : axis == 1 ? mine.y : mine.z;
                        const float q1 = s1 - __builtin_amdgcn_fmed3f(s1, lo1, hi1);
                        const float q2 = s2 - __builtin_amdgcn_fmed3f(s2, lo2, hi2);
                        const float b2_lo = FUSED ? __builtin_fmaf(q1, q1, q2 * q2) : q1 * q1 + q2 * q2;
                        bool keep = !(b2_lo >= mine.w);
                        unsigned long long rest = __builtin_amdgcn_ballot_w64(keep) & m_mask;
                        keep = __builtin_amdgcn_inverse_ballot_w64(rest);
                        if (rest != 0ull && __builtin_amdgcn_ballot_w64(keep && mine.w < lat_r2) != 0ull) {
                            float p1 = INFINITY, p2 = INFINITY;
                            for (int k = 0; k < 8; ++k) {
                                p1 = fminf(p1, fabsf(s1 - s_lat[wv][0][k]));
                                p2 = fminf(p2, fabsf(s2 - s_lat[wv][1][k]));
                            }
                            const float nan_if_nan = (s1 + s2) * 0.0f;
                            const float l2 = (FUSED ? __builtin_fmaf(p1, p1, p2 * p2) : p1 * p1 + p2 * p2) + nan_if_nan;
                            keep = keep && !(l2 >= mine.w);
                            rest = __builtin_amdgcn_ballot_w64(keep);
                        }
                        if (rest == 0ull) continue;
                        const unsigned long long inside =
                            __builtin_amdgcn_ballot_w64(__builtin_fmaf(sa, da0, noda_lo) >= 0.0f)
                            & __builtin_amdgcn_ballot_w64(__builtin_fmaf(sa, da0, noda_hi) < len_lo);
                        const bool lean = same_sense && (rest & ~inside) == 0ull;
                        const bool fat = FUSED && (rest & ~__builtin_amdgcn_ballot_w64(mine.w >= fat_r2)) == 0ull;
                        const int cls = (c >> (GRANULE_SHIFT - 6)) & (SUM_CLASSES - 1);
                        const int n = __builtin_amdgcn_readlane(cnt, cls);
                        const int bits = (lean ? 1 : 0) | (fat ? 2 : 0);
                        const int n_surv = __builtin_popcountll(rest);
                        const int open_n = __builtin_amdgcn_readlane(round_n, cls);
                        const int open_bits = __builtin_amdgcn_readlane(round_bits, cls);
                        const bool close_cap = n > 0 && open_n + n_surv > 64;
                        const bool close_flag = n > 0 && !close_cap && open_bits != bits;
                        const bool close = close_cap || close_flag;
                        if (pl.spans) {
                            const int4 span = pl.spans[packet * SUM_CLASSES + cls];
                            const int surv_at = __builtin_amdgcn_readlane(t_surv, cls);
                            const int closed = __builtin_amdgcn_readlane(t_rounds, cls);
                            if (surv_at + n_surv <= span.z && closed + (close ? 1 : 0) < span.w) {
                                if (close && lane == 0) pl.hdr[size_t(span.y) + closed] = plan_header(open_n, open_bits);
                                if ((rest >> lane) & 1ull)
                                    pl.idx[size_t(span.x) + surv_at
                                           + int(__builtin_amdgcn_mbcnt_hi(uint32_t(rest >> 32),
                                                                           __builtin_amdgcn_mbcnt_lo(uint32_t(rest), 0u)))] =
                                        uint32_t(pbase + lane);
                            } else {
                                failed = true;
                            }
                        }
                        if (lane == cls) {
                            if (close) {
                                t_rounds += 1; t_full += open_n == 64 ? 1 : 0;
                                t_cap += close_cap ? 1 : 0; t_flag += close_flag ? 1 : 0;
                                t_max = max(t_max, open_n);
                                round_closed(open_n, open_bits);
                                round_n = 0;
                            }
                            round_n += n_surv; round_bits = bits;
                            t_surv += n_surv;
                            cnt += 1;
                        }
                    }
                }
            }
        }
    }
    if (failed) {
        cnt = 0;
        if (lane == 0) { pl.ctl->unusable = 1u; pl.ctl->usable = 0u; }
    }
    if (lane < SUM_CLASSES && cnt > 0) {
        if (pl.spans && !failed)
            pl.hdr[size_t(pl.spans[packet * SUM_CLASSES + lane].y) + t_rounds] = plan_header(round_n, round_bits);
        t_rounds += 1; t_full += round_n == 64 ? 1 : 0;
        t_max = max(t_max, round_n);
        round_closed(round_n, round_bits);
        t_loops += 1; t_lmax = max(t_lmax, loop_n);
    }
    if (lane < SUM_CLASSES) pl.counts[packet * SUM_CLASSES + lane] = failed ? make_int4(0, 0, 0, 0) : make_int4(t_rounds, t_surv, cnt, 0);
    if (pl.spans && !failed) {
        if (lane >= SUM_CLASSES) cnt = 0;
        int tally[7] = { cnt, t_surv, t_rounds, t_full, t_cap, t_flag, t_loops };
#pragma unroll
        for (int off = 1; off < SUM_CLASSES; off <<= 1) {
#pragma unroll
            for (int k = 0; k < 7; ++k) tally[k] += __shfl_xor(tally[k], off);
            t_max = max(t_max, __shfl_xor(t_max, off));
            t_lmax = max(t_lmax, __shfl_xor(t_lmax, off));
        }
        if (lane == 0) {
#pragma unroll
            for (int k = 0; k < 6; ++k)
                if (tally[k]) atomicAdd(&pl.ctl->stats[k], (unsigned long long)tally[k]);
            if (tally[6]) atomicAdd(&pl.ctl->loops, (unsigned long long)tally[6]);
            atomicMax(&pl.ctl->largest_round, uint32_t(t_max));
            atomicMax(&pl.ctl->largest_loop, uint32_t(t_lmax));
        }
    }
}

grace_status launch_record(const bool fast, const TraceArgs& a, const PlanRef& pl, hipStream_t stream)
{
    const int n_packets = (a.n_rays + a.width - 1) / a.width;
    const int grid = ceil_div(size_t(n_packets), size_t(TRACE_BLOCK / 64));
    if (fast) plan_record_kernel<true><<<grid, TRACE_BLOCK, 0, stream>>>(a, pl);
    else plan_record_kernel<false><<<grid, TRACE_BLOCK, 0, stream>>>(a, pl);
    GRACE_CHECK_LAUNCH();
    return GRACE_OK;
}

grace_status plan_free_buffers(PacketPlan& pp)
{
    void* bufs[] = { pp.idx, pp.hdr, pp.spans, pp.counts, pp.ctl };
    bool any = false;
    for (void* b : bufs) any = any || b;
    if (any) GRACE_TRY_HIP(hipDeviceSynchronize());
    for (void* b : bufs)
        if (b) GRACE_TRY_HIP(hipFree(b));
    pp.idx = nullptr; pp.hdr = nullptr; pp.spans = nullptr; pp.counts = nullptr; pp.ctl = nullptr;
    pp.valid = false;
    pp.n_lists = pp.n_words = pp.n_hdrs = pp.recorded = 0;
    return GRACE_OK;
}

}

namespace grace_hip {

grace_status plan_release(TraceState& ts)
{
    GRACE_TRY(plan_free_buffers(ts.plan));
    ts.plan = PacketPlan();
    ts.last_plan_ctl = nullptr;
    return GRACE_OK;
}

grace_status plan_fill(TraceState& ts, const PlanKey& key, const TraceArgs& a, hipStream_t stream)
{
    PacketPlan& pp = ts.plan;
    GRACE_TRY(plan_free_buffers(pp));
    ts.last_plan_ctl = nullptr;
    pp.key = key;
    pp.dead = true;
    const int n_packets = (a.n_rays + a.width - 1) / a.width;
    const size_t n_lists = size_t(n_packets) * SUM_CLASSES;
    auto alloc = [&](auto*& ptr, const size_t bytes) {
        if (hipMalloc(reinterpret_cast<void**>(&ptr), bytes) == hipSuccess) return true;
        (void)hipGetLastError();
        ptr = nullptr;
        return false;
    };
    if (n_lists * (sizeof(int4) + sizeof(int4)) > ts.plan_budget) return GRACE_OK;
    if (!alloc(pp.counts, n_lists * sizeof(int4)) || !alloc(pp.spans, n_lists * sizeof(int4))
        || !alloc(pp.ctl, sizeof(PlanCtl)))
        return plan_free_buffers(pp);
    GRACE_TRY_HIP(hipMemsetAsync(pp.ctl, 0, sizeof(PlanCtl), stream));
    GRACE_TRY(launch_record(key.fast, a, PlanRef{ nullptr, nullptr, nullptr, pp.counts, pp.ctl, 1 }, stream));
    std::vector<int4> counts(n_lists);
    PlanCtl seen = {};
    GRACE_TRY_HIP(hipMemcpyAsync(counts.data(), pp.counts, n_lists * sizeof(int4), hipMemcpyDeviceToHost, stream));
    GRACE_TRY_HIP(hipMemcpyAsync(&seen, pp.ctl, sizeof(seen), hipMemcpyDeviceToHost, stream));
    GRACE_TRY_HIP(hipStreamSynchronize(stream));
    if (seen.unusable) return plan_free_buffers(pp);
    std::vector<int4> spans(n_lists);
    size_t words = 0, hdrs = 0, used = 0;
    for (size_t l = 0; l < n_lists; ++l) {
        const size_t surv = size_t(counts[l].y), entries = size_t(counts[l].z);
        const size_t room_s = surv + surv / 8 + 2, room_r = entries + entries / 8 + 2;
        spans[l] = make_int4(int(words), int(hdrs), int(room_s), int(room_r));
        words += room_s;
        hdrs += room_r;
        used += surv;
        if (words >= (size_t(1) << 31) - PLAN_IDX_PAD) return plan_free_buffers(pp);
    }
    pp.n_lists = n_lists; pp.n_words = words; pp.n_hdrs = hdrs; pp.recorded = used;
    if (pp.bytes() > ts.plan_budget || !alloc(pp.idx, (words + PLAN_IDX_PAD) * sizeof(uint32_t))
        || !alloc(pp.hdr, (hdrs + PLAN_HDR_PAD) * sizeof(uint32_t)))
        return plan_free_buffers(pp);
    GRACE_TRY_HIP(hipMemcpy(pp.spans, spans.data(), n_lists * sizeof(int4), hipMemcpyHostToDevice));
    GRACE_TRY_HIP(hipMemsetAsync(pp.idx + words, 0, PLAN_IDX_PAD * sizeof(uint32_t), stream));
    GRACE_TRY_HIP(hipMemsetAsync(pp.hdr + hdrs, 0, PLAN_HDR_PAD * sizeof(uint32_t), stream));
    GRACE_TRY_HIP(hipMemsetD32Async(reinterpret_cast<hipDeviceptr_t>(&pp.ctl->usable), 1, 1, stream));
    GRACE_TRY_HIP(hipMemcpyAsync(&pp.ctl->sig[0], ts.scene.ctl->sig, 16, hipMemcpyDeviceToDevice, stream));
    GRACE_TRY_HIP(hipMemcpyAsync(&pp.ctl->sig[2], ts.rays.ctl->sig, 16, hipMemcpyDeviceToDevice, stream));
    GRACE_TRY(launch_record(key.fast, a, PlanRef{ pp.idx, pp.hdr, pp.spans, pp.counts, pp.ctl, 1 }, stream));
    pp.valid = true;
    pp.dead = false;
    return GRACE_OK;
}

grace_status plan_record(const TraceState& ts, const TraceArgs& a, hipStream_t stream)
{
    const PacketPlan& pp = ts.plan;
    return launch_record(pp.key.fast, a, PlanRef{ pp.idx, pp.hdr, pp.spans, pp.counts, pp.ctl, 0 }, stream);
}

grace_status launch_planned(const int mode, const bool fast, const int grid, const TraceArgs& a, hipStream_t stream)
{
    auto go = [&](auto mode_tag) {
        constexpr int MODE = decltype(mode_tag)::value;
        if (fast) trace_kernel<MODE, true, true, false, true><<<grid, TRACE_BLOCK, 0, stream>>>(a);
        else trace_kernel<MODE, true, false, false, true><<<grid, TRACE_BLOCK, 0, stream>>>(a);
    };
    switch (mode) {
    case MODE_CUMULATIVE: go(std::integral_constant<int, MODE_CUMULATIVE>()); break;
    case MODE_WCUM1: go(std::integral_constant<int, MODE_WCUM1>()); break;
    case MODE_WCUM2: go(std::integral_constant<int, MODE_WCUM2>()); break;
    case MODE_WCUM3: go(std::integral_constant<int, MODE_WCUM3>()); break;
    case MODE_WCUM4: go(std::integral_constant<int, MODE_WCUM4>()); break;
    default: return set_error(GRACE_INVALID_ARGUMENT, __FILE__, __LINE__, "no planned kernel for this mode");
    }
    GRACE_CHECK_LAUNCH();
    return GRACE_OK;
}

}
```

grace-devel_amd/csrc/trace_prepass.hip:

```cpp
#include "trace_state.hpp"

using namespace grace_hip;

namespace {

__device__ __forceinline__ float cluster_box_of_wave(const float4 s, const bool have, const size_t c,
                                                     float4* __restrict__ C)
{
    const int lane = threadIdx.x & 63;
    float lo[3] = { INFINITY, INFINITY, INFINITY }, hi[3] = { -INFINITY, -INFINITY, -INFINITY };
    float r2_min = INFINITY;
    if (have) {
        r2_min = s.w;
        const float r = sqrtf(s.w) * 1.00001f;
        const float ctr[3] = { s.x, s.y, s.z };
#pragma unroll
        for (int k = 0; k < 3; ++k) {
            const float slack = (fabsf(ctr[k]) + r) * 4.76837158203125e-07f;
            lo[k] = (ctr[k] - r) - slack;
            hi[k] = (ctr[k] + r) + slack;
        }
    }
#pragma unroll
    for (int k = 0; k < 3; ++k) {
#pragma unroll
        for (int off = 32; off > 0; off >>= 1) {
            lo[k] = fminf(lo[k], __shfl_xor(lo[k], off));
            hi[k] = fmaxf(hi[k], __shfl_xor(hi[k], off));
        }
    }
#pragma unroll
    for (int off = 32; off > 0; off >>= 1) r2_min = fminf(r2_min, __shfl_xor(r2_min, off));
    if (lane == 0) {
        C[2 * c] = make_float4(lo[0], lo[1], lo[2], r2_min);
        C[2 * c + 1] = make_float4(hi[0], hi[1], hi[2], 0.f);
    }
    return r2_min;
}

__device__ __forceinline__ void publish_r2_min(const float wave_r2_min, float4* __restrict__ C_tail)
{
    __shared__ float s_r2_min[4];
    if ((threadIdx.x & 63) == 0) s_r2_min[(threadIdx.x >> 6) & 3] = wave_r2_min;
    __syncthreads();
    if (threadIdx.x == 0) {
        float m = s_r2_min[0];
        for (unsigned w = 1; w < blockDim.x / 64 && w < 4; ++w) m = fminf(m, s_r2_min[w]);
        if (m < INFINITY) atomicMin(reinterpret_cast<unsigned int*>(C_tail), __float_as_uint(m));
    }
}

__global__ __launch_bounds__(256) void trace_prepass_kernel(const float4* __restrict__ spheres,
                                                            size_t n, float4* __restrict__ A,
                                                            float2* __restrict__ B1,
                                                            float2* __restrict__ B50,
                                                            float4* __restrict__ C,
                                                            const uint32_t* __restrict__ run_if)
{
    if (run_if && *run_if == 0u) return;
    float wave_r2_min = INFINITY;
    for (size_t i = blockIdx.x * size_t(blockDim.x) + threadIdx.x; (i & ~size_t(63)) < n + 4;
         i += size_t(gridDim.x) * blockDim.x) {

        float4 a = make_float4(0.f, 0.f, 0.f, 0.f);
        float2 b1 = make_float2(0.f, 0.f), b50 = b1;
        if (i < n) {
            const float4 s = spheres[i];
            a = make_float4(s.x, s.y, s.z, s.w * s.w);
            const float ir = 1.f / s.w;
            b1 = make_float2(ir, ir * ir);
            b50 = make_float2(ir * float(N_TABLE - 1), fminf(ir * ir, 3.4028234664e38f));
        }
        if (i < n + 4) {
            A[i] = a;
            if (B1) B1[i] = b1;
            if (B50) B50[i] = b50;
        }
        if (C && (i & ~size_t(63)) < n) wave_r2_min = fminf(wave_r2_min, cluster_box_of_wave(a, i < n, i >> 6, C));
    }
    if (C) publish_r2_min(wave_r2_min, C + 2 * ((n + 63) / 64));
}

__global__ __launch_bounds__(256) void trace_prepass_d4_kernel(const double* __restrict__ spheres,
                                                               size_t n, float4* __restrict__ A)
{
    for (size_t i = blockIdx.x * size_t(blockDim.x) + threadIdx.x; i < n + 4;
         i += size_t(gridDim.x) * blockDim.x) {
        float4 a = make_float4(0.f, 0.f, 0.f, 0.f);
        if (i < n) {
            const double* s = spheres + 4 * i;
            const double r = fabs(s[3]) * (1.0 + 3.814697265625e-06)
                + (fabs(s[0]) + fabs(s[1]) + fabs(s[2]) + fabs(s[3])) * 4.76837158203125e-07;
            a = make_float4(float(s[0]), float(s[1]), float(s[2]), float(r * r * (1.0 + 1e-6)));
        }
        A[i] = a;
    }
}

__global__ __launch_bounds__(256) void trace_prepass_f4d_kernel(const float4* __restrict__ spheres,
                                                                size_t n, float4* __restrict__ A)
{
    for (size_t i = blockIdx.x * size_t(blockDim.x) + threadIdx.x; i < n + 4;
         i += size_t(gridDim.x) * blockDim.x) {
        float4 a = make_float4(0.f, 0.f, 0.f, 0.f);
        if (i < n) {
            const float4 s = spheres[i];
            const double w = s.w;
            a = make_float4(s.x, s.y, s.z, float(w * w * (1.0 + 1.52587890625e-05 )));
        }
        A[i] = a;
    }
}

__global__ __launch_bounds__(256) void cluster_boxes_kernel(const float4* __restrict__ A, size_t n,
                                                            float4* __restrict__ C,
                                                            const uint32_t* __restrict__ run_if)
{
    if (run_if && *run_if == 0u) return;
    const size_t n_clusters = (n + 63) / 64;
    const int lane = threadIdx.x & 63;
    float wave_r2_min = INFINITY;
    for (size_t c = blockIdx.x * size_t(blockDim.x / 64) + (threadIdx.x >> 6); c < n_clusters;
         c += size_t(gridDim.x) * (blockDim.x / 64)) {
        const size_t i = c * 64 + lane;
        const bool have = i < n;
        const float4 s = have ? A[i] : make_float4(0.f, 0.f, 0.f, 0.f);
        wave_r2_min = fminf(wave_r2_min, cluster_box_of_wave(s, have, c, C));
    }
    publish_r2_min(wave_r2_min, C + 2 * n_clusters);
}

__global__ __launch_bounds__(256) void group_boxes_kernel(const float4* __restrict__ C, size_t n_clusters,
                                                          int per_group, size_t n_groups,
                                                          float4* __restrict__ G,
                                                          const uint32_t* __restrict__ run_if)
{
    if (run_if && *run_if == 0u) return;
    const int lane = threadIdx.x & 63;
    for (size_t g = blockIdx.x * size_t(blockDim.x / 64) + (threadIdx.x >> 6); g < n_groups;
         g += size_t(gridDim.x) * (blockDim.x / 64)) {
        float lo[3] = { INFINITY, INFINITY, INFINITY }, hi[3] = { -INFINITY, -INFINITY, -INFINITY };
        const size_t c0 = g * size_t(per_group);
        for (size_t c = c0 + lane; c < c0 + per_group && c < n_clusters; c += 64) {
            const float4 l = C[2 * c], h = C[2 * c + 1];
            lo[0] = fminf(lo[0], l.x); lo[1] = fminf(lo[1], l.y); lo[2] = fminf(lo[2], l.z);
            hi[0] = fmaxf(hi[0], h.x); hi[1] = fmaxf(hi[1], h.y); hi[2] = fmaxf(hi[2], h.z);
        }
#pragma unroll
        for (int k = 0; k < 3; ++k) {
#pragma unroll
            for (int off = 32; off > 0; off >>= 1) {
                lo[k] = fminf(lo[k], __shfl_xor(lo[k], off));
                hi[k] = fmaxf(hi[k], __shfl_xor(hi[k], off));
            }
        }
// ... 186 lines not shown
```

grace-devel_amd/csrc/trace_state.hpp:

```cpp
#pragma once

#include "common.hpp"

namespace grace_hip {

constexpr int TRACE_BLOCK = 256;
constexpr int N_TABLE = 51;
constexpr int SPLIT_WIDE_BUDGET = 0x100;

inline int group_shift(size_t n_prims)
{
    int s = 12;
    while (((n_prims + (size_t(1) << s) - 1) >> s) > 4096) ++s;
    return s;
}
inline size_t group_count(size_t n_prims)
{
    const int s = group_shift(n_prims);
    return (n_prims + (size_t(1) << s) - 1) >> s;
}
inline size_t cluster_record_count(size_t n_prims)
{
    return 2 * ((n_prims + 63) / 64) + 1 + 2 * group_count(n_prims);
}
// ... 95 lines not shown
    const int4* wave_map;
    const int* n_wave_map;
    bool keep_chunks;
    int chunk_shift, n_chunks;
    int width;
    const float4* nodes;
    int n_nodes;
    const int4* leaves;
    const int* root;
    int* out_counts;
    float* out_sums;
    const int* offsets;
    int* hit_idx;
    float* hit_integral;
    float* hit_dist;
    uint32_t* stats;
    int* status;
    const float* weights;
    int w_stride;
    int out_stride;
    const double* kernel_table;
    const uint32_t* plan_idx;
    const int4* plan_spans;
    const int4* plan_counts;
    const uint32_t* plan_usable;
    const int* plan_split_dev;
    const uint32_t* plan_hdr;
};


struct CacheCtl {
    unsigned long long sig[2];
    uint32_t stale;
    uint32_t pad;
};

struct SceneKey {
    Primitive kind = PRIM_F4;
    const void* prims = nullptr; const void* nodes = nullptr; const void* leaves = nullptr;
    size_t n_prims = 0, n_nodes = 0;
    bool operator==(const SceneKey& o) const
    {
        return kind == o.kind && prims == o.prims && nodes == o.nodes && leaves == o.leaves
            && n_prims == o.n_prims && n_nodes == o.n_nodes;
    }
};

struct Scene {
    bool valid = false;
    SceneKey key;
    SceneKey seen;
    float4* A = nullptr; float2* B1 = nullptr; float2* B50 = nullptr; double* T64 = nullptr;
    int2* node_prims = nullptr; float4* C = nullptr;
    CacheCtl* ctl = nullptr;
    bool pinned = false;
    unsigned long long gen = 0;
};

struct RayKey {
    const float* rays = nullptr;
    size_t n = 0;
    bool operator==(const RayKey& o) const { return rays == o.rays && n == o.n; }
};

struct RayOrder {
    bool valid = false;
    RayKey key, seen;
    uint32_t* perm = nullptr;
    uint32_t* ext = nullptr;
    CacheCtl* ctl = nullptr;
    bool pinned = false;
    unsigned long long gen = 0;
};

struct PlanCtl {
    uint32_t record;
    uint32_t unusable;
    uint32_t usable;
    uint32_t largest_round;
    unsigned long long sig[4];
    unsigned long long stats[6];
    unsigned long long loops;
    uint32_t largest_loop, pad;
};
constexpr int PLAN_FORMAT = 3;
__host__ __device__ inline uint32_t plan_header(const int n_surv, const int bits)
{
    return uint32_t(n_surv) | (uint32_t(bits) << 8);
}
__host__ __device__ inline int plan_header_count(const uint32_t h) { return int(h & 0xffu) < 64 ? int(h & 0xffu) : 64; }
__host__ __device__ inline int plan_header_bits(const uint32_t h) { return int((h >> 8) & 3u); }
constexpr size_t PLAN_IDX_PAD = 128, PLAN_HDR_PAD = 8;

struct PlanKey {
    int format = PLAN_FORMAT;
    bool fast = false;
    int group_shift = 0, width = 0;
    bool reorder = false;
    size_t n_rays = 0, n_prims = 0;
    unsigned long long scene_gen = 0, rays_gen = 0;
    bool operator==(const PlanKey& o) const
    {
        return format == o.format && fast == o.fast && group_shift == o.group_shift && width == o.width && reorder == o.reorder
            && n_rays == o.n_rays && n_prims == o.n_prims && scene_gen == o.scene_gen && rays_gen == o.rays_gen;
    }
};

struct PacketPlan {
    bool valid = false;
    bool dead = false;
    PlanKey key;
    uint32_t* idx = nullptr;
    uint32_t* hdr = nullptr;
    int4* spans = nullptr;
    int4* counts = nullptr;
    PlanCtl* ctl = nullptr;
    size_t n_lists = 0, n_words = 0, n_hdrs = 0;
    size_t recorded = 0;
    size_t bytes() const
    {
        return (n_words + PLAN_IDX_PAD + n_hdrs + PLAN_HDR_PAD) * sizeof(uint32_t)
            + n_lists * (sizeof(int4) + sizeof(int4)) + sizeof(PlanCtl);
    }
};

struct PlanGate {
    const CacheCtl* scene = nullptr;
    const CacheCtl* rays = nullptr;
    PlanCtl* ctl = nullptr;
};

__host__ __device__ inline int planned_split(const int n_packets)
{
    return n_packets <= 8192 ? SUM_CLASSES : SUM_CLASSES / 2;
}

constexpr int PLAN_LOOP_MAX = 128;
__host__ __device__ inline bool planned_fuses(const int loop_n, const int loop_bits, const uint32_t next)
{
    return (loop_bits & 1) != 0 && plan_header_bits(next) == loop_bits
        && loop_n + plan_header_count(next) <= PLAN_LOOP_MAX;
}

struct HitsCache {
    int* chunk_counts = nullptr;
    size_t capacity = 0;
    bool valid = false;
    const void* rays = nullptr; const void* prims = nullptr;
    size_t n_rays = 0, n_prims = 0;
    int n_chunks = 0;
};

struct TraceState {
    int* status = nullptr;
    const int* last_lat_dev = nullptr;
    hipStream_t last_lat_stream = nullptr;
    bool timing = false;
    hipEvent_t ev0 = nullptr, ev1 = nullptr;
    bool ev_valid = false;
    bool ray_reorder = true;
    int treelet = -1;
    int split = -1;
    int lat_split = 4;
    int width = -1;
    bool exact_integrals = false;
    bool hits_stage_split = true;
    bool cache_validation = true;
    bool cache_auto = true;
    int sph_kernel = 0;
    const double* builtin_tables = nullptr;
    const double* kernel_table = nullptr;
    double* custom_table = nullptr;
    double custom_host[N_TABLE] = {};
    bool plan_on = true;
    size_t plan_budget = size_t(512) << 20;
    Scene scene;
    RayOrder rays;
    HitsCache hits;
    unsigned long long cache_gen = 0;
    PacketPlan plan;
    const PlanCtl* last_plan_ctl = nullptr;
    hipStream_t last_plan_stream = nullptr;
    bool last_plan_fuses = false;
};

grace_status trace_state(TraceState** out);

inline grace_status ensure_status(TraceState& ts, hipStream_t stream)
{
    if (!ts.status) {
        GRACE_TRY_HIP(hipMalloc(reinterpret_cast<void**>(&ts.status), sizeof(int)));
        GRACE_TRY_HIP(hipMemsetAsync(ts.status, 0, sizeof(int), stream));
    }
    return GRACE_OK;
}

template <typename Launches>
grace_status timed(TraceState& ts, hipStream_t stream, Launches launches)
{
    if (ts.timing) {
        if (!ts.ev0) { GRACE_TRY_HIP(hipEventCreate(&ts.ev0)); GRACE_TRY_HIP(hipEventCreate(&ts.ev1)); }
        GRACE_TRY_HIP(hipEventRecord(ts.ev0, stream));
    }
    GRACE_TRY(launches());
    if (ts.timing) {
        GRACE_TRY_HIP(hipEventRecord(ts.ev1, stream));
        ts.ev_valid = true;
    }
    return GRACE_OK;
}

size_t sig_partial_words();
struct SigRequest {
    const void* prims = nullptr; size_t prims_bytes = 0;
    const void* nodes = nullptr; size_t nodes_bytes = 0;
    const void* leaves = nullptr; size_t leaves_bytes = 0;
    CacheCtl* scene_ctl = nullptr; bool scene_force = false;
    const void* rays = nullptr; size_t rays_bytes = 0;
    CacheCtl* rays_ctl = nullptr; bool rays_force = false;
    uint32_t* rays_ext = nullptr;
};
grace_status launch_signatures(const SigRequest& rq, unsigned long long* partial, hipStream_t stream);

grace_status scene_release(TraceState& ts);
grace_status scene_cache_alloc(TraceState& ts, const SceneKey& key);
grace_status scene_fill(Primitive kind, const void* prims, size_t n_prims, const float4* nodes,
                        size_t n_nodes, const int4* leaves, float4* A, float2* B1, float2* B50,
                        double* T64, int2* node_prims, float4* C, hipStream_t stream,
                        const uint32_t* run_if = nullptr);
grace_status scene_prepare(TraceState& ts, Primitive kind, const void* prims, size_t n_prims,
                           const int* d_nodes, size_t n_nodes, const int* d_leaves, hipStream_t stream);

grace_status rays_release(TraceState& ts);
grace_status rays_cache_alloc(TraceState& ts, const RayKey& key);
grace_status ray_order(const float* d_rays, size_t n_rays, uint32_t* ext, uint32_t* keys, uint32_t* perm,
                       const float4* scene_min, uint32_t* lat_flag, int n_packets, int split, int* split_dev,
                       hipStream_t stream, const uint32_t* run_if = nullptr);
grace_status rays_prepare(TraceState& ts, const float* d_rays, size_t n_rays, hipStream_t stream);
grace_status launch_choose_variants(const uint32_t* ext12, int n, const float4* scene_min, uint32_t* lat_flag,
                                    int split_packets, int split_launched, int* split_dev, hipStream_t stream,
                                    const PlanGate* gate = nullptr, int* plan_split_dev = nullptr);

grace_status plan_release(TraceState& ts);
grace_status plan_fill(TraceState& ts, const PlanKey& key, const TraceArgs& a, hipStream_t stream);
grace_status plan_record(const TraceState& ts, const TraceArgs& a, hipStream_t stream);
grace_status launch_planned(int mode, bool fast, int grid, const TraceArgs& a, hipStream_t stream);

}
```

grace-devel_amd/grace_hip/__init__.py:

```python
import collections
import ctypes as C
import os

import numpy as np
import torch

_HERE = os.path.dirname(os.path.abspath(__file__))
LIB_PATH = os.path.join(os.path.dirname(_HERE), "lib", "libgrace_hip.so")

if not os.path.exists(LIB_PATH):
    raise ImportError(
        "libgrace_hip.so is not built (%s). Run __graft_entry__.build() or "
        "`make -C grace-devel_amd`. There is no CPU fallback." % LIB_PATH)

_lib = C.CDLL(LIB_PATH)
_lib.grace_last_error.restype = C.c_char_p
_lib.grace_version.restype = C.c_int

GRACE_OK = 0
GRACE_INVALID_ARGUMENT = 1
GRACE_HIP_ERROR = 2
GRACE_OUT_OF_MEMORY = 3
GRACE_STACK_OVERFLOW = 4

# ... 263 lines not shown


def set_exact_integrals(enabled):
    _check(_lib.grace_trace_set_exact_integrals(C.c_int(1 if enabled else 0)))


SPH_KERNELS = ("cubic", "quartic", "quintic", "wendland_c2", "wendland_c4", "wendland_c6")
SPH_KERNEL_CUSTOM = -1


def _kernel_kind(name):
    if name not in SPH_KERNELS:
        raise ValueError("unknown SPH kernel %r (one of %s)" % (name, ", ".join(SPH_KERNELS)))
    return SPH_KERNELS.index(name)


def sph_kernel_table(name):
    out = (C.c_double * N_TABLE)()
    _check(_lib.grace_sph_kernel_table(C.c_int(_kernel_kind(name)), out))
    return np.array(out, np.float64)


def set_sph_kernel(kernel):
    if isinstance(kernel, str):
        _check(_lib.grace_trace_set_sph_kernel(C.c_int(_kernel_kind(kernel))))
        return
    t = np.asarray(kernel)
    if t.dtype.kind not in "fiu" or t.ndim != 1:
        raise ValueError("an SPH kernel table must be a 1-D array of 51 numbers")
    t = np.ascontiguousarray(t, dtype=np.float64)
    _check(_lib.grace_trace_set_sph_kernel_table(t.ctypes.data_as(C.POINTER(C.c_double)), C.c_int(len(t))))


def sph_kernel():
    kind = C.c_int(0)
    out = (C.c_double * N_TABLE)()
    _check(_lib.grace_trace_get_sph_kernel(C.byref(kind), out))
    name = "custom" if kind.value == SPH_KERNEL_CUSTOM else SPH_KERNELS[kind.value]
    return name, np.array(out, np.float64)


def set_cache_validation(enabled):
    _check(_lib.grace_trace_set_cache_validation(C.c_int(1 if enabled else 0)))


def set_cache_auto(enabled):
    _check(_lib.grace_trace_set_cache_auto(C.c_int(1 if enabled else 0)))


def set_plan(enabled):
    _check(_lib.grace_trace_set_plan(C.c_int(1 if enabled else 0)))


def set_plan_budget(n_bytes):
    _check(_lib.grace_trace_set_plan_budget(C.c_size_t(int(n_bytes))))


def plan_bytes():
    v = C.c_size_t(0)
    _check(_lib.grace_trace_plan_bytes(C.byref(v)))
    return v.value


def last_plan_used():
    v = C.c_int(0)
    _check(_lib.grace_trace_last_plan_used(C.byref(v)))
    return v.value


PlanStats = collections.namedtuple(
    "PlanStats", "entries survivors rounds full_rounds closed_by_capacity closed_by_flags largest_round")


def plan_stats():
    v = (C.c_ulonglong * 7)()
    _check(_lib.grace_trace_plan_stats(v))
    return PlanStats(*[int(x) for x in v])


def plan_loops():
    v = (C.c_ulonglong * 2)()
    _check(_lib.grace_trace_plan_loops(v))
    return int(v[0]), int(v[1])


def set_lattice_split(k):
    _check(_lib.grace_trace_set_lattice_split(C.c_int(k)))


def set_hits_staging(enabled):
    _check(_lib.grace_trace_set_hits_staging(C.c_int(1 if enabled else 0)))


class Context:

    def __init__(self):
        self._h = C.c_void_p(0)
        _check(_lib.grace_context_create(C.byref(self._h)))

    def make_current(self):
        _check(_lib.grace_context_set_current(self._h))

    @staticmethod
    def reset_current():
        _check(_lib.grace_context_set_current(C.c_void_p(0)))

    def destroy(self):
        if self._h:
            _check(_lib.grace_context_destroy(self._h))
            self._h = C.c_void_p(0)

    def __enter__(self):
        self.make_current()
        return self

    def __exit__(self, *exc):
        Context.reset_current()
        self.destroy()
        return False


def set_treelet_size(n):
    _check(_lib.grace_trace_set_treelet_size(C.c_int(int(n))))


def set_ray_reorder(enabled):
    _check(_lib.grace_trace_set_ray_reorder(C.c_int(1 if enabled else 0)))


def trace_status():
    _check(_lib.grace_trace_status(_stream()))


_prepared = {}


def trace_prepare(spheres, tree):
    _check(_lib.grace_trace_prepare_f4(_ptr(_spheres(spheres)), C.c_size_t(len(spheres)),
                                       _ptr(tree.nodes), C.c_size_t(tree.n_nodes),
                                       _ptr(tree.leaves), _stream()))
    _prepared["scene"] = (spheres, tree.nodes, tree.leaves)


def trace_prepare_tri(tris, tree):
    _check(_lib.grace_trace_prepare_tri(_ptr(_tris(tris)), C.c_size_t(len(tris)),
                                        _ptr(tree.nodes), C.c_size_t(tree.n_nodes),
                                        _ptr(tree.leaves), _stream()))
    _prepared["scene"] = (tris, tree.nodes, tree.leaves)


def trace_prepare_rays(rays):
    _check(_lib.grace_trace_prepare_rays(_ptr(_rays(rays)), C.c_size_t(len(rays)), _stream()))
    _prepared["rays"] = rays


def trace_release_rays():
    _check(_lib.grace_trace_release_rays())
    _prepared.pop("rays", None)


def trace_release():
    _check(_lib.grace_trace_release())
    _prepared.pop("scene", None)


def _trace_hitcounts_keep(rays, spheres, tree, hit_counts, real=torch.float32):
# ... 1165 lines not shown
```

include/grace_hip.h:

```cpp
#ifndef GRACE_HIP_H
#define GRACE_HIP_H

#include <stddef.h>
#include <stdint.h>

#ifdef __cplusplus
extern "C" {
#endif

typedef enum grace_status {
    GRACE_OK = 0,
    GRACE_INVALID_ARGUMENT = 1,
    GRACE_HIP_ERROR = 2,
    GRACE_OUT_OF_MEMORY = 3,
    GRACE_STACK_OVERFLOW = 4
} grace_status;

typedef void* grace_stream;

int grace_version(void);
const char* grace_last_error(void);

grace_status grace_device_malloc(void** d_ptr, size_t bytes);
grace_status grace_device_free(void* d_ptr);
// ... 136 lines not shown
    double v0;
    double dv;
    int    n_bins;
    int    periodic;
    double hubble;
} grace_spectrum_grid;
grace_status grace_trace_spectra_f4(const void* d_rays, size_t n_rays, const float* d_spheres,
                                    size_t n_spheres, const int* d_nodes, size_t n_nodes,
                                    const int* d_leaves, const int* d_root,
                                    const float* d_amount, const float* d_width, const float* d_velocity,
                                    int n_channels, const grace_spectrum_grid* grid, float* d_tau,
                                    float* d_column, grace_stream stream);
grace_status grace_trace_set_ordered_budget(size_t bytes);
grace_status grace_trace_ordered_limits(int* wave_max_hits, int* block_max_hits);
typedef struct grace_ordered_stats {
    unsigned long long batches;
    unsigned long long total_hits;
    unsigned long long rays_wave, rays_block, rays_global;
    unsigned long long budget_bytes, frame_bytes;
    float ms_count, ms_trace, ms_composite;
} grace_ordered_stats;
grace_status grace_trace_ordered_enable_stats(int enabled);
grace_status grace_trace_ordered_last_stats(grace_ordered_stats* h_stats);
grace_status grace_trace_hits_f4(const void* d_rays, size_t n_rays, const float* d_spheres,
                                 size_t n_spheres, const int* d_nodes, size_t n_nodes,
                                 const int* d_leaves, const int* d_root,
                                 const int* d_ray_offsets, int* d_hit_indices,
                                 float* d_hit_integrals, float* d_hit_distances,
                                 grace_stream stream);
grace_status grace_trace_stats_f4(const void* d_rays, size_t n_rays, const float* d_spheres,
                                  size_t n_spheres, const int* d_nodes, size_t n_nodes,
                                  const int* d_leaves, const int* d_root,
                                  uint32_t* d_stats4, grace_stream stream);

grace_status grace_hit_integrals_f32(const float* d_b2, const float* d_h, size_t n, float* d_out,
                                     grace_stream stream);

grace_status grace_trace_set_ray_reorder(int enabled);

grace_status grace_trace_enable_timing(int enabled);
grace_status grace_trace_last_kernel_ms(float* h_ms);

grace_status grace_trace_last_lattice(int* h_lattice);

grace_status grace_trace_set_packet_split(int waves_per_packet);

grace_status grace_trace_set_packet_width(int rays_per_packet);

grace_status grace_trace_set_exact_integrals(int enabled);

#define GRACE_SPH_KERNEL_CUSTOM      (-1)
#define GRACE_SPH_KERNEL_CUBIC       0
#define GRACE_SPH_KERNEL_QUARTIC     1
#define GRACE_SPH_KERNEL_QUINTIC     2
#define GRACE_SPH_KERNEL_WENDLAND_C2 3
#define GRACE_SPH_KERNEL_WENDLAND_C4 4
#define GRACE_SPH_KERNEL_WENDLAND_C6 5
grace_status grace_trace_set_sph_kernel(int kind);
grace_status grace_trace_set_sph_kernel_table(const double* h_table, int n);
grace_status grace_trace_get_sph_kernel(int* h_kind, double* h_table51);
grace_status grace_sph_kernel_table(int kind, double* h_out51);

grace_status grace_trace_set_treelet_size(int max_primitives);

grace_status grace_trace_set_lattice_split(int waves_per_packet);
grace_status grace_trace_set_hits_staging(int enabled);

grace_status grace_trace_prepare_f4(const float* d_spheres, size_t n_spheres, const int* d_nodes,
                                    size_t n_nodes, const int* d_leaves, grace_stream stream);
grace_status grace_trace_prepare_tri(const float* d_tris, size_t n_tris, const int* d_nodes,
                                     size_t n_nodes, const int* d_leaves, grace_stream stream);
grace_status grace_trace_release(void);
grace_status grace_trace_prepare_rays(const void* d_rays, size_t n_rays, grace_stream stream);
grace_status grace_trace_release_rays(void);
grace_status grace_trace_set_cache_validation(int enabled);
grace_status grace_trace_set_cache_auto(int enabled);

grace_status grace_trace_set_plan(int on);
grace_status grace_trace_set_plan_budget(size_t bytes);
grace_status grace_trace_plan_bytes(size_t* h_bytes);
grace_status grace_trace_last_plan_used(int* h_used);
grace_status grace_trace_plan_stats(unsigned long long* h_stats );
grace_status grace_trace_plan_loops(unsigned long long* h_loops );

grace_status grace_trace_status(grace_stream stream);

grace_status grace_scan_exclusive_i32(const int* d_in, size_t n, int* d_out, long long* h_total,
                                      grace_stream stream);
grace_status grace_segscan_exclusive_f32(const int* d_segment_offsets, size_t n_segments,
                                         const float* d_data, size_t n, float* d_results,
                                         grace_stream stream);
grace_status grace_segscan_exclusive_f64(const int* d_segment_offsets, size_t n_segments,
                                         const double* d_data, size_t n, double* d_results,
                                         grace_stream stream);
grace_status grace_add_iota_i32(int* d_values, size_t n, grace_stream stream);
grace_status grace_fill_u32(void* d_values, size_t n, uint32_t bits, grace_stream stream);
grace_status grace_multiply_by_weights_f32(const float* d_unweighted, size_t n,
                                           const float* d_weights, const uint32_t* d_weight_map,
                                           float* d_weighted, grace_stream stream);
grace_status grace_multiply_by_weights_f64(const double* d_unweighted, size_t n,
                                           const double* d_weights, const uint32_t* d_weight_map,
                                           double* d_weighted, grace_stream stream);

grace_status grace_sort_by_distance_f32(float* d_distances, const int* d_ray_offsets,
                                        size_t n_rays, size_t n_hits, int* d_hit_indices,
                                        float* d_hit_data, grace_stream stream);

grace_status grace_sort_by_distance_f64(double* d_distances, const int* d_ray_offsets,
                                        size_t n_rays, size_t n_hits, int* d_hit_indices,
                                        double* d_hit_data, grace_stream stream);

grace_status grace_rays_orthogonal_z(int n_side, const float* h_mins4, const float* h_maxs4,
                                     void* d_rays, float* h_area, grace_stream stream);
grace_status grace_rays_pinhole(int res_x, int res_y, const float* h_camera, const float* h_look_at,
                                const float* h_view_up, float fovy, float length, void* d_rays,
                                grace_stream stream);
grace_status grace_rays_healpix(int nside, float ox, float oy, float oz, float length,
                                void* d_rays, grace_stream stream);
grace_status grace_rays_isotropic(size_t n_rays, float ox, float oy, float oz, float length,
                                  uint64_t seed, void* d_rays, grace_stream stream);

grace_status grace_rays_isotropic_octant(size_t n_rays, float ox, float oy, float oz, float length,
                                         int octant, uint64_t seed, void* d_rays,
                                         grace_stream stream);
grace_status grace_rays_one_to_many(size_t n_rays, float ox, float oy, float oz,
                                    const void* d_points, int is_double, int elems_per_point,
                                    int sort_type, const float* h_bot, const float* h_top,
                                    void* d_rays, grace_stream stream);
grace_status grace_rays_plane_parallel_random(int width, int height, const float* h_base,
                                              const float* h_w, const float* h_h, float length,
                                              uint64_t seed, void* d_rays, grace_stream stream);
grace_status grace_rays_orthographic_projection(int res_x, int res_y, const float* h_camera,
                                                const float* h_look_at, const float* h_view_up,
                                                float vertical_extent, float length,
                                                void* d_rays, grace_stream stream);

grace_status grace_deltas_euclid_d4(const double* d_spheres, size_t n, float* d_deltas,
                                    grace_stream stream);
grace_status grace_deltas_euclid_d4_f64(const double* d_spheres, size_t n, double* d_deltas,
                                        grace_stream stream);
grace_status grace_deltas_area_d4(const double* d_spheres, size_t n, float* d_deltas,
                                  grace_stream stream);
grace_status grace_deltas_area_d4_f64(const double* d_spheres, size_t n, double* d_deltas,
                                      grace_stream stream);
grace_status grace_albvh_build_f4_u64(const float* d_spheres, size_t n, const uint64_t* d_deltas,
                                      int max_per_leaf, int* d_nodes, int* d_leaves, int* d_root,
                                      size_t* h_n_leaves, grace_stream stream);
grace_status grace_albvh_build_f4_f64(const float* d_spheres, size_t n, const double* d_deltas,
                                      int max_per_leaf, int* d_nodes, int* d_leaves, int* d_root,
                                      size_t* h_n_leaves, grace_stream stream);
grace_status grace_albvh_build_d4_f64(const double* d_spheres, size_t n, const double* d_deltas,
                                      int max_per_leaf, int* d_nodes, int* d_leaves, int* d_root,
                                      size_t* h_n_leaves, grace_stream stream);
grace_status grace_albvh_build_d4_u32(const double* d_spheres, size_t n, const uint32_t* d_deltas,
                                      int max_per_leaf, int* d_nodes, int* d_leaves, int* d_root,
                                      size_t* h_n_leaves, grace_stream stream);
grace_status grace_albvh_build_d4_u64(const double* d_spheres, size_t n, const uint64_t* d_deltas,
                                      int max_per_leaf, int* d_nodes, int* d_leaves, int* d_root,
                                      size_t* h_n_leaves, grace_stream stream);
grace_status grace_albvh_build_d4(const double* d_spheres, size_t n, const float* d_deltas,
                                  int max_per_leaf, int* d_nodes, int* d_leaves, int* d_root,
                                  size_t* h_n_leaves, grace_stream stream);
grace_status grace_trace_hitcounts_d4(const void* d_rays, size_t n_rays, const double* d_spheres,
                                      size_t n_spheres, const int* d_nodes, size_t n_nodes,
                                      const int* d_leaves, const int* d_root, int* d_hit_counts,
                                      grace_stream stream);
// ... 199 lines not shown
```

Baseline: 576.5.

## Add sub-tile packet plans splitting each wave into four quadrant survivor lists

The plan recorder now builds separate survivor lists for each 16-lane quadrant of a ray packet. It culls each primitive against the quadrant's origin bounds and interleaves the indices four-wide, padding with a sentinel primitive. The fused planned kernel reads its tile with a per-quadrant offset and stride of four, so each quadrant steps only through its own survivors. The intent is to cut wasted integral steps when survivors hit only part of the packet. In exchange it adds padding slots, a larger LDS tile, bank-pattern changes on the reads, and more complex plan recording with new API controls.

After: 622.6, median of 6. 1.08x the previous value.

```diff
diff --git a/grace-devel_amd/csrc/trace.hip b/grace-devel_amd/csrc/trace.hip
--- a/grace-devel_amd/csrc/trace.hip
+++ b/grace-devel_amd/csrc/trace.hip
@@ -124,6 +124,7 @@
     uint32_t* ext = nullptr; uint32_t* keys = nullptr; uint32_t* perm = nullptr;
     bool plan_eligible = false;
     PlanKey plan_key;
+    int plan_request = 0;
 };
 
 template <int MODE>
@@ -154,8 +155,15 @@
     const bool scene_cached = scene_use != USE_NONE, rays_cached = rays_use != USE_NONE;
     auto held = [](const CacheUse u) { return u == USE_CHECK || u == USE_TRUST; };
     b.plan_eligible = ts.plan_on && f4_sums(MODE) && held(scene_use) && held(rays_use) && p.lat_split == 0;
-    if (b.plan_eligible)
-        b.plan_key = PlanKey{ PLAN_FORMAT, p.fast_b, group_shift(n_prims), p.width, p.reorder, n_rays, n_prims, ts.scene.gen, ts.rays.gen };
+    if (b.plan_eligible) {
+        b.plan_key = PlanKey{ PLAN_FORMAT, false, p.fast_b, group_shift(n_prims), p.width, p.reorder, n_rays, n_prims, ts.scene.gen, ts.rays.gen };
+        b.plan_request = !weighted(MODE) && p.fast_b && p.width == 64 ? ts.plan_subtiles : 0;
+        if (b.plan_request != 0) {
+            const PacketPlan& pp = ts.plan;
+            const bool answered = (pp.valid || pp.dead) && pp.key == b.plan_key && pp.asked == b.plan_request;
+            b.plan_key.subtiles = !answered;
+        }
+    }
     PlanGate gate;
     const bool plan_steady = b.plan_eligible && ts.plan.valid && ts.plan.key == b.plan_key;
     if (plan_steady) {
@@ -303,7 +311,7 @@
                 GRACE_TRY(plan_record(ts, a, stream));
                 const int grid_planned = a.plan_split_dev
                     ? ceil_div(size_t(p.n_packets) * planned_split(p.n_packets), TRACE_BLOCK / 64) : grid;
-                GRACE_TRY(launch_planned(MODE, ALT, grid_planned, a, stream));
+                GRACE_TRY(launch_planned(MODE, ALT, ts.plan.key.subtiles, grid_planned, a, stream));
                 if (p.split == 1) GRACE_TRY(combine(1, nullptr, reinterpret_cast<const int*>(a.plan_usable)));
             }
             if (p.split > 1) launch_walk<MODE, true, ALT>(grid, a, stream);
@@ -404,7 +412,8 @@
     if constexpr (f4_sums(MODE)) {
         PacketPlan& pp = ts.plan;
         if (b.plan_eligible && !(pp.key == b.plan_key && (pp.valid || pp.dead)))
-            GRACE_TRY(plan_fill(ts, b.plan_key, a, stream));
+            GRACE_TRY(plan_fill(ts, b.plan_key, b.plan_request, a, stream));
+        if (b.plan_eligible && (pp.valid || pp.dead) && pp.asked == b.plan_request) b.plan_key.subtiles = pp.key.subtiles;
         ts.last_plan_ctl = nullptr;
         if (b.plan_eligible && pp.valid && pp.key == b.plan_key) {
             a.plan_idx = pp.idx; a.plan_hdr = pp.hdr; a.plan_spans = pp.spans; a.plan_counts = pp.counts;
@@ -847,6 +856,29 @@
     return GRACE_OK;
 }
 
+grace_status grace_trace_set_plan_subtiles(int mode)
+{
+    GRACE_REQUIRE(mode >= -1 && mode <= 1, "plan sub-tiles: -1 (automatic), 0 (never) or 1 (whenever eligible)");
+    GRACE_TRACE_STATE();
+    if (ts.plan_subtiles != mode) GRACE_TRY(plan_release(ts));
+    ts.plan_subtiles = mode;
+    return GRACE_OK;
+}
+
+grace_status grace_trace_plan_subtiles(int* h_used, unsigned long long* h_steps, unsigned long long* h_slots)
+{
+    GRACE_REQUIRE(h_used && h_steps && h_slots, "null output");
+    *h_used = 0; *h_steps = 0; *h_slots = 0;
+    GRACE_TRACE_STATE();
+    if (ts.last_plan_ctl && ts.plan.valid && ts.plan.key.subtiles) {
+        PlanCtl h = {};
+        GRACE_TRY_HIP(hipStreamSynchronize(ts.last_plan_stream));
+        GRACE_TRY_HIP(hipMemcpy(&h, ts.last_plan_ctl, sizeof(h), hipMemcpyDeviceToHost));
+        if (h.usable != 0u) { *h_used = 1; *h_steps = h.sub_steps; *h_slots = h.sub_slots; }
+    }
+    return GRACE_OK;
+}
+
 grace_status grace_trace_plan_bytes(size_t* h_bytes)
 {
     GRACE_REQUIRE(h_bytes, "null output");
diff --git a/grace-devel_amd/csrc/trace_coherence.hip b/grace-devel_amd/csrc/trace_coherence.hip
--- a/grace-devel_amd/csrc/trace_coherence.hip
+++ b/grace-devel_amd/csrc/trace_coherence.hip
@@ -191,6 +191,7 @@
             for (int k = 0; k < 6; ++k) pc.stats[k] = 0ull;
             pc.largest_round = 0u;
             pc.loops = 0ull; pc.largest_loop = 0u;
+            pc.sub_steps = 0ull; pc.sub_slots = 0ull;
         }
     }
 }
diff --git a/grace-devel_amd/csrc/trace_kernel.hpp b/grace-devel_amd/csrc/trace_kernel.hpp
--- a/grace-devel_amd/csrc/trace_kernel.hpp
+++ b/grace-devel_amd/csrc/trace_kernel.hpp
@@ -236,7 +236,7 @@
     __device__ WeightedB(const float2 b) : x(b.x), y(b.y), w{} {}
 };
 
-template <int MODE, bool SPLIT, bool ALT = false, bool LAT = false, bool PLANNED = false>
+template <int MODE, bool SPLIT, bool ALT = false, bool LAT = false, bool PLANNED = false, bool SUBTILE = false>
 __global__ __launch_bounds__(TRACE_BLOCK, !f4_class_split(MODE) ? 1
                                           : weighted(MODE) ? (channels(MODE) == 1 ? 6 : 7 - channels(MODE))
                                           : (SPLIT ? 8 : 6))
@@ -257,13 +257,16 @@
     constexpr int NW = channels(MODE), WP = WEIGHTED ? (NW + 1) / 2 : 0;
     using BRec = std::conditional_t<WEIGHTED, WeightedB<NW>, float2>;
     constexpr bool FUSE = PLANNED && !WEIGHTED && FAST;
+    static_assert(!SUBTILE || FUSE, "sub-tile plans: the unweighted fast planned kernel only");
+    constexpr int STEP = SUBTILE ? 4 : 1;
     __shared__ double2 s_lut[FAST ? 1 : N_TABLE];
     constexpr int LUTF_N = 256;
     __shared__ float2 s_lutf[FAST ? LUTF_N : 1];
     constexpr bool D4 = primitive(MODE) == PRIM_D4, F4D = primitive(MODE) == PRIM_F4D;
     constexpr bool LDS_TILE = primitive(MODE) == PRIM_F4;
-    __shared__ __align__(16) float2 s_tile[LDS_TILE ? TRACE_BLOCK / 64 : 1][LDS_TILE ? (FUSE ? 4 : 3 + WP) : 1][LDS_TILE ? 66 : 1];
-    static_assert(!FUSE || 4 * 66 * sizeof(float2) >= (PLAN_LOOP_MAX + 2) * sizeof(float4), "the fused loop's tile");
+    constexpr int TILE_SLOTS = SUBTILE ? 68 : 66;
+    __shared__ __align__(16) float2 s_tile[LDS_TILE ? TRACE_BLOCK / 64 : 1][LDS_TILE ? (FUSE ? 4 : 3 + WP) : 1][LDS_TILE ? TILE_SLOTS : 1];
+    static_assert(!FUSE || 4 * TILE_SLOTS * sizeof(float2) >= (PLAN_LOOP_MAX + 2 * STEP) * sizeof(float4), "the fused loop's tile");
     __shared__ double s_tile_d[D4 ? TRACE_BLOCK / 64 : 1][D4 ? 64 : 1][D4 ? 6 : 1];
     __shared__ float4 s_tile_f[F4D ? TRACE_BLOCK / 64 : 1][F4D ? 64 : 1][F4D ? 2 : 1];
     const int lane = threadIdx.x & 63;
@@ -796,7 +799,7 @@
                     if constexpr (PLANNED) {
                         round_n_next = loop_n;
                         round_bits_next = uint32_t(loop_bits);
-                        const int pj = int(min(plan_word, uint32_t(r_hi - 1)));
+                        const int pj = int(min(plan_word, uint32_t(SUBTILE ? r_hi : r_hi - 1)));
                         mine_next = a.A[pj];
                         if (NEED_B) mineb_next = a.B[pj];
                         if constexpr (WEIGHTED) {
@@ -805,7 +808,7 @@
                         }
                         if constexpr (FUSE) {
                             if (loop_n > 64) {
-                                const int pj2 = int(min(plan_word2, uint32_t(r_hi - 1)));
+                                const int pj2 = int(min(plan_word2, uint32_t(SUBTILE ? r_hi : r_hi - 1)));
                                 mine2_next = a.A[pj2];
                                 mine2b_next = a.B[pj2];
                             }
@@ -1109,6 +1112,7 @@
                     int at;
                     if (COMPACT) {
                         at = k++;
+                        if constexpr (SUBTILE) at = 4 * at + (lane >> 4);
                         jj = 0;
                     } else {
                         at = __builtin_ctzll(td);
@@ -1141,6 +1145,7 @@
                     BRec b0 = make_float2(0.f, 0.f), b1 = b0, b2 = b0;
                     int j0, j1 = 0, j2 = 0;
                     int left = __builtin_popcountll(todo);
+                    if constexpr (SUBTILE) left = max(round_n >> 2, 1);
                     unsigned long long td = todo | 0x8000000000000000ull;
                     int k = 0;
                     fetch(td, k, c0, b0, j0);
@@ -1162,6 +1167,7 @@
                     float4 c0, c1, c2;
                     int left = FUSE ? round_n : __builtin_popcountll(todo);
                     const float4* t4 = tile4;
+                    if constexpr (SUBTILE) { left = max(round_n >> 2, 1); t4 = tile4 + (lane >> 4); }
                     if constexpr (WEIGHTED && NW > 1) {
                         float4 x0, x1;
                         auto procw = [&](const float4 c, const float4 x) {
@@ -1195,18 +1201,18 @@
                         else sum = __builtin_fmaf(__builtin_fmaf(y.y, b, y.x), c.w, sum);
                     };
                     c0 = t4[0]; __builtin_amdgcn_sched_barrier(0);
-                    c1 = t4[1]; __builtin_amdgcn_sched_barrier(0);
+                    c1 = t4[STEP]; __builtin_amdgcn_sched_barrier(0);
                     for (;;) {
-                        c2 = t4[2]; __builtin_amdgcn_sched_barrier(0);
+                        c2 = t4[2 * STEP]; __builtin_amdgcn_sched_barrier(0);
                         proc(c0);
                         if (--left == 0) break;
-                        c0 = t4[3]; __builtin_amdgcn_sched_barrier(0);
+                        c0 = t4[3 * STEP]; __builtin_amdgcn_sched_barrier(0);
                         proc(c1);
                         if (--left == 0) break;
-                        c1 = t4[4]; __builtin_amdgcn_sched_barrier(0);
+                        c1 = t4[4 * STEP]; __builtin_amdgcn_sched_barrier(0);
                         proc(c2);
                         if (--left == 0) break;
-                        t4 += 3;
+                        t4 += 3 * STEP;
                     }
                 };
                 if constexpr (LEAN4) {
diff --git a/grace-devel_amd/csrc/trace_planned.hip b/grace-devel_amd/csrc/trace_planned.hip
--- a/grace-devel_amd/csrc/trace_planned.hip
+++ b/grace-devel_amd/csrc/trace_planned.hip
@@ -15,9 +15,10 @@
     int force;
 };
 
-template <bool FUSED>
+template <bool FUSED, bool SUB = false>
 __global__ __launch_bounds__(TRACE_BLOCK) void plan_record_kernel(const TraceArgs a, const PlanRef pl)
 {
+    static_assert(!SUB || FUSED, "sub-tile plans: the fast integral only");
     __shared__ float s_lat[TRACE_BLOCK / 64][2][8];
     if (pl.spans && !pl.force && pl.ctl->record == 0u) return;
     const int lane = threadIdx.x & 63, wv = threadIdx.x >> 6;
@@ -32,6 +33,8 @@
     int round_n = 0, round_bits = 0;
     int t_surv = 0, t_rounds = 0, t_full = 0, t_cap = 0, t_flag = 0, t_max = 0;
     int loop_n = 0, loop_bits = 0, t_loops = 0, t_lmax = 0;
+    int sub_pos = 0, sub_touched = 0;
+    (void)sub_pos; (void)sub_touched;
     auto round_closed = [&](const int n, const int bits) {
         if (FUSED && loop_n > 0 && planned_fuses(loop_n, loop_bits, plan_header(n, bits))) {
             loop_n += n;
@@ -54,6 +57,26 @@
         float cell2;
         build_origin_lattice(ar.o1, ar.o2, lane, s_lat, lat_ok, cell2);
         const float lat_r2 = lat_ok ? cell2 : 0.f;
+        float qlo1[4] = {}, qhi1[4] = {}, qlo2[4] = {}, qhi2[4] = {};
+        unsigned long long q_lanes[4] = {};
+        if constexpr (SUB) {
+            float m1 = ray.valid ? ar.o1 : INFINITY, x1 = ray.valid ? ar.o1 : -INFINITY;
+            float m2 = ray.valid ? ar.o2 : INFINITY, x2 = ray.valid ? ar.o2 : -INFINITY;
+#pragma unroll
+            for (int off = 1; off < 16; off <<= 1) {
+                m1 = fminf(m1, __shfl_xor(m1, off)); x1 = fmaxf(x1, __shfl_xor(x1, off));
+                m2 = fminf(m2, __shfl_xor(m2, off)); x2 = fmaxf(x2, __shfl_xor(x2, off));
+            }
+            const unsigned long long valid_lanes = __builtin_amdgcn_ballot_w64(ray.valid);
+#pragma unroll
+            for (int q = 0; q < 4; ++q) {
+                qlo1[q] = __builtin_bit_cast(float, __builtin_amdgcn_readlane(__builtin_bit_cast(int, m1), 16 * q));
+                qhi1[q] = __builtin_bit_cast(float, __builtin_amdgcn_readlane(__builtin_bit_cast(int, x1), 16 * q));
+                qlo2[q] = __builtin_bit_cast(float, __builtin_amdgcn_readlane(__builtin_bit_cast(int, m2), 16 * q));
+                qhi2[q] = __builtin_bit_cast(float, __builtin_amdgcn_readlane(__builtin_bit_cast(int, x2), 16 * q));
+                q_lanes[q] = ((valid_lanes >> (16 * q)) & 0xffffull) != 0ull ? ~0ull : 0ull;
+            }
+        }
 
         auto box_may_hit = [&](const float4 blo, const float4 bhi, const bool along) {
             const float l1 = axis == 0 ? blo.y : blo.x, h1 = axis == 0 ? bhi.y : bhi.x;
@@ -120,6 +143,41 @@
                         const int n = __builtin_amdgcn_readlane(cnt, cls);
                         const int bits = (lean ? 1 : 0) | (fat ? 2 : 0);
                         const int n_surv = __builtin_popcountll(rest);
+                        if constexpr (SUB) {
+                            const int4 span = pl.spans ? pl.spans[packet * SUM_CLASSES + cls] : make_int4(0, 0, 0, 0);
+                            int touched = __builtin_amdgcn_readlane(sub_touched, cls);
+#pragma unroll
+                            for (int q = 0; q < 4; ++q) {
+                                const float u1 = s1 - __builtin_amdgcn_fmed3f(s1, qlo1[q], qhi1[q]);
+                                const float u2 = s2 - __builtin_amdgcn_fmed3f(s2, qlo2[q], qhi2[q]);
+                                const unsigned long long rest_q =
+                                    __builtin_amdgcn_ballot_w64(!(__builtin_fmaf(u1, u1, u2 * u2) >= mine.w)) & rest & q_lanes[q];
+                                if (rest_q == 0ull) continue;
+                                const int n_q = __builtin_popcountll(rest_q);
+                                const int at = __builtin_amdgcn_readlane(sub_pos, 4 * cls + q);
+                                const int r_first = at / PLAN_SUB_ROUND_STEPS, r_last = (at + n_q - 1) / PLAN_SUB_ROUND_STEPS;
+                                if (pl.spans) {
+                                    if (at + n_q <= span.z && r_last < span.w) {
+                                        if ((rest_q >> lane) & 1ull)
+                                            pl.idx[size_t(span.x) + 4 * size_t(at + int(__builtin_amdgcn_mbcnt_hi(uint32_t(rest_q >> 32),
+                                                                                           __builtin_amdgcn_mbcnt_lo(uint32_t(rest_q), 0u)))) + q] =
+                                                uint32_t(pbase + lane);
+                                        if (lane == 0) {
+                                            for (int r = r_first; r <= r_last; ++r) {
+                                                uint32_t* const h = pl.hdr + size_t(span.y) + r;
+                                                *h = plan_header(64, r < touched ? bits & plan_header_bits(*h) : bits);
+                                            }
+                                        }
+                                    } else {
+                                        failed = true;
+                                    }
+                                }
+                                touched = max(touched, r_last + 1);
+                                if (lane == 4 * cls + q) sub_pos += n_q;
+                            }
+                            if (lane == cls) { sub_touched = touched; t_surv += n_surv; cnt += 1; }
+                            continue;
+                        }
                         const int open_n = __builtin_amdgcn_readlane(round_n, cls);
                         const int open_bits = __builtin_amdgcn_readlane(round_bits, cls);
                         const bool close_cap = n > 0 && open_n + n_surv > 64;
@@ -161,7 +219,49 @@
         cnt = 0;
         if (lane == 0) { pl.ctl->unusable = 1u; pl.ctl->usable = 0u; }
     }
-    if (lane < SUM_CLASSES && cnt > 0) {
+    int sub_steps = 0, sub_real = 0;
+    if constexpr (SUB) {
+        for (int c = 0; c < SUM_CLASSES; ++c) {
+            int steps = 0, real = 0;
+#pragma unroll
+            for (int q = 0; q < 4; ++q) {
+                const int n = failed ? 0 : __builtin_amdgcn_readlane(sub_pos, 4 * c + q);
+                steps = max(steps, n); real += n;
+            }
+            const int rounds = (steps + PLAN_SUB_ROUND_STEPS - 1) / PLAN_SUB_ROUND_STEPS;
+            int loops = 0, lmax = 0;
+            if (pl.spans && steps > 0) {
+                const int4 span = pl.spans[packet * SUM_CLASSES + c];
+#pragma unroll
+                for (int q = 0; q < 4; ++q)
+                    for (int t = __builtin_amdgcn_readlane(sub_pos, 4 * c + q) + lane; t < steps; t += 64)
+                        pl.idx[size_t(span.x) + 4 * size_t(t) + q] = uint32_t(a.n_prims);
+                if (lane == 0) {
+                    uint32_t* const h = pl.hdr + size_t(span.y);
+                    h[rounds - 1] = plan_header(4 * (steps - (rounds - 1) * PLAN_SUB_ROUND_STEPS), plan_header_bits(h[rounds - 1]));
+                    int ln = 0, lb = 0;
+                    for (int r = 0; r < rounds; ++r) {
+                        const uint32_t next = h[r];
+                        if (ln > 0 && planned_fuses(ln, lb, next)) {
+                            ln += plan_header_count(next);
+                        } else {
+                            if (ln > 0) { loops += 1; lmax = max(lmax, ln); }
+                            ln = plan_header_count(next); lb = plan_header_bits(next);
+                        }
+                    }
+                    loops += 1; lmax = max(lmax, ln);
+                }
+                loops = __builtin_amdgcn_readlane(loops, 0); lmax = __builtin_amdgcn_readlane(lmax, 0);
+            }
+            if (lane == c) {
+                t_rounds = rounds; t_full = steps / PLAN_SUB_ROUND_STEPS;
+                t_max = min(4 * steps, 4 * PLAN_SUB_ROUND_STEPS);
+                t_loops = loops; t_lmax = lmax;
+                sub_steps = steps; sub_real = real;
+            }
+        }
+    }
+    if (!SUB && lane < SUM_CLASSES && cnt > 0) {
         if (pl.spans && !failed)
             pl.hdr[size_t(pl.spans[packet * SUM_CLASSES + lane].y) + t_rounds] = plan_header(round_n, round_bits);
         t_rounds += 1; t_full += round_n == 64 ? 1 : 0;
@@ -169,7 +269,7 @@
         round_closed(round_n, round_bits);
         t_loops += 1; t_lmax = max(t_lmax, loop_n);
     }
-    if (lane < SUM_CLASSES) pl.counts[packet * SUM_CLASSES + lane] = failed ? make_int4(0, 0, 0, 0) : make_int4(t_rounds, t_surv, cnt, 0);
+    if (lane < SUM_CLASSES) pl.counts[packet * SUM_CLASSES + lane] = failed ? make_int4(0, 0, 0, 0) : make_int4(t_rounds, t_surv, cnt, sub_steps);
     if (pl.spans && !failed) {
         if (lane >= SUM_CLASSES) cnt = 0;
         int tally[7] = { cnt, t_surv, t_rounds, t_full, t_cap, t_flag, t_loops };
@@ -179,23 +279,27 @@
             for (int k = 0; k < 7; ++k) tally[k] += __shfl_xor(tally[k], off);
             t_max = max(t_max, __shfl_xor(t_max, off));
             t_lmax = max(t_lmax, __shfl_xor(t_lmax, off));
+            if constexpr (SUB) { sub_steps += __shfl_xor(sub_steps, off); sub_real += __shfl_xor(sub_real, off); }
         }
         if (lane == 0) {
 #pragma unroll
             for (int k = 0; k < 6; ++k)
                 if (tally[k]) atomicAdd(&pl.ctl->stats[k], (unsigned long long)tally[k]);
             if (tally[6]) atomicAdd(&pl.ctl->loops, (unsigned long long)tally[6]);
+            if (SUB && sub_steps) atomicAdd(&pl.ctl->sub_steps, (unsigned long long)sub_steps);
+            if (SUB && sub_real) atomicAdd(&pl.ctl->sub_slots, (unsigned long long)sub_real);
             atomicMax(&pl.ctl->largest_round, uint32_t(t_max));
             atomicMax(&pl.ctl->largest_loop, uint32_t(t_lmax));
         }
     }
 }
 
-grace_status launch_record(const bool fast, const TraceArgs& a, const PlanRef& pl, hipStream_t stream)
+grace_status launch_record(const bool fast, const bool subtiles, const TraceArgs& a, const PlanRef& pl, hipStream_t stream)
 {
     const int n_packets = (a.n_rays + a.width - 1) / a.width;
     const int grid = ceil_div(size_t(n_packets), size_t(TRACE_BLOCK / 64));
-    if (fast) plan_record_kernel<true><<<grid, TRACE_BLOCK, 0, stream>>>(a, pl);
+    if (subtiles) plan_record_kernel<true, true><<<grid, TRACE_BLOCK, 0, stream>>>(a, pl);
+    else if (fast) plan_record_kernel<true><<<grid, TRACE_BLOCK, 0, stream>>>(a, pl);
     else plan_record_kernel<false><<<grid, TRACE_BLOCK, 0, stream>>>(a, pl);
     GRACE_CHECK_LAUNCH();
     return GRACE_OK;
@@ -212,6 +316,7 @@
     pp.idx = nullptr; pp.hdr = nullptr; pp.spans = nullptr; pp.counts = nullptr; pp.ctl = nullptr;
     pp.valid = false;
     pp.n_lists = pp.n_words = pp.n_hdrs = pp.recorded = 0;
+    pp.key.subtiles = false;
     return GRACE_OK;
 }
 
@@ -227,12 +332,14 @@
     return GRACE_OK;
 }
 
-grace_status plan_fill(TraceState& ts, const PlanKey& key, const TraceArgs& a, hipStream_t stream)
+grace_status plan_fill(TraceState& ts, const PlanKey& key, const int request, const TraceArgs& a, hipStream_t stream)
 {
     PacketPlan& pp = ts.plan;
     GRACE_TRY(plan_free_buffers(pp));
     ts.last_plan_ctl = nullptr;
     pp.key = key;
+    pp.key.subtiles = false;
+    pp.asked = request;
     pp.dead = true;
     const int n_packets = (a.n_rays + a.width - 1) / a.width;
     const size_t n_lists = size_t(n_packets) * SUM_CLASSES;
@@ -246,49 +353,73 @@
     if (!alloc(pp.counts, n_lists * sizeof(int4)) || !alloc(pp.spans, n_lists * sizeof(int4))
         || !alloc(pp.ctl, sizeof(PlanCtl)))
         return plan_free_buffers(pp);
-    GRACE_TRY_HIP(hipMemsetAsync(pp.ctl, 0, sizeof(PlanCtl), stream));
-    GRACE_TRY(launch_record(key.fast, a, PlanRef{ nullptr, nullptr, nullptr, pp.counts, pp.ctl, 1 }, stream));
-    std::vector<int4> counts(n_lists);
-    PlanCtl seen = {};
-    GRACE_TRY_HIP(hipMemcpyAsync(counts.data(), pp.counts, n_lists * sizeof(int4), hipMemcpyDeviceToHost, stream));
-    GRACE_TRY_HIP(hipMemcpyAsync(&seen, pp.ctl, sizeof(seen), hipMemcpyDeviceToHost, stream));
-    GRACE_TRY_HIP(hipStreamSynchronize(stream));
-    if (seen.unusable) return plan_free_buffers(pp);
-    std::vector<int4> spans(n_lists);
-    size_t words = 0, hdrs = 0, used = 0;
-    for (size_t l = 0; l < n_lists; ++l) {
-        const size_t surv = size_t(counts[l].y), entries = size_t(counts[l].z);
-        const size_t room_s = surv + surv / 8 + 2, room_r = entries + entries / 8 + 2;
-        spans[l] = make_int4(int(words), int(hdrs), int(room_s), int(room_r));
-        words += room_s;
-        hdrs += room_r;
-        used += surv;
-        if (words >= (size_t(1) << 31) - PLAN_IDX_PAD) return plan_free_buffers(pp);
-    }
-    pp.n_lists = n_lists; pp.n_words = words; pp.n_hdrs = hdrs; pp.recorded = used;
-    if (pp.bytes() > ts.plan_budget || !alloc(pp.idx, (words + PLAN_IDX_PAD) * sizeof(uint32_t))
-        || !alloc(pp.hdr, (hdrs + PLAN_HDR_PAD) * sizeof(uint32_t)))
-        return plan_free_buffers(pp);
-    GRACE_TRY_HIP(hipMemcpy(pp.spans, spans.data(), n_lists * sizeof(int4), hipMemcpyHostToDevice));
-    GRACE_TRY_HIP(hipMemsetAsync(pp.idx + words, 0, PLAN_IDX_PAD * sizeof(uint32_t), stream));
-    GRACE_TRY_HIP(hipMemsetAsync(pp.hdr + hdrs, 0, PLAN_HDR_PAD * sizeof(uint32_t), stream));
-    GRACE_TRY_HIP(hipMemsetD32Async(reinterpret_cast<hipDeviceptr_t>(&pp.ctl->usable), 1, 1, stream));
-    GRACE_TRY_HIP(hipMemcpyAsync(&pp.ctl->sig[0], ts.scene.ctl->sig, 16, hipMemcpyDeviceToDevice, stream));
-    GRACE_TRY_HIP(hipMemcpyAsync(&pp.ctl->sig[2], ts.rays.ctl->sig, 16, hipMemcpyDeviceToDevice, stream));
-    GRACE_TRY(launch_record(key.fast, a, PlanRef{ pp.idx, pp.hdr, pp.spans, pp.counts, pp.ctl, 1 }, stream));
-    pp.valid = true;
-    pp.dead = false;
+    std::vector<int4> counts(n_lists), spans(n_lists);
+    for (int sub = request != 0 && key.fast && a.width == 64 ? 1 : 0; sub >= 0; --sub) {
+        GRACE_TRY_HIP(hipMemsetAsync(pp.ctl, 0, sizeof(PlanCtl), stream));
+        GRACE_TRY(launch_record(key.fast, sub != 0, a, PlanRef{ nullptr, nullptr, nullptr, pp.counts, pp.ctl, 1 }, stream));
+        PlanCtl seen = {};
+        GRACE_TRY_HIP(hipMemcpyAsync(counts.data(), pp.counts, n_lists * sizeof(int4), hipMemcpyDeviceToHost, stream));
+        GRACE_TRY_HIP(hipMemcpyAsync(&seen, pp.ctl, sizeof(seen), hipMemcpyDeviceToHost, stream));
+        GRACE_TRY_HIP(hipStreamSynchronize(stream));
+        if (seen.unusable) return plan_free_buffers(pp);
+        size_t words = 0, hdrs = 0, used = 0, steps = 0;
+        bool fits = true;
+        for (size_t l = 0; l < n_lists && fits; ++l) {
+            const size_t surv = size_t(counts[l].y), entries = size_t(counts[l].z), len = size_t(counts[l].w);
+            const size_t room_s = sub ? len + len / 8 + 2 : surv + surv / 8 + 2;
+            const size_t room_r = sub ? (room_s + PLAN_SUB_ROUND_STEPS - 1) / PLAN_SUB_ROUND_STEPS : entries + entries / 8 + 2;
+            spans[l] = make_int4(int(words), int(hdrs), int(room_s), int(room_r));
+            words += sub ? 4 * room_s : room_s;
+            hdrs += room_r;
+            used += surv;
+            steps += len;
+            fits = words < (size_t(1) << 31) - PLAN_IDX_PAD;
+        }
+        pp.n_lists = n_lists; pp.n_words = words; pp.n_hdrs = hdrs; pp.recorded = used;
+        fits = fits && pp.bytes() <= ts.plan_budget;
+        if (sub) {
+            const bool pays = n_packets >= PLAN_SUB_MIN_PACKETS && double(steps) < PLAN_SUB_MAX_RATIO * double(used);
+            if (!fits || (request < 0 && !pays)) continue;
+        }
+        if (!fits || !alloc(pp.idx, (words + PLAN_IDX_PAD) * sizeof(uint32_t))
+            || !alloc(pp.hdr, (hdrs + PLAN_HDR_PAD) * sizeof(uint32_t))) {
+            if (sub) {
+                if (pp.idx) { GRACE_TRY_HIP(hipFree(pp.idx)); pp.idx = nullptr; }
+                continue;
+            }
+            return plan_free_buffers(pp);
+        }
+        GRACE_TRY_HIP(hipMemcpy(pp.spans, spans.data(), n_lists * sizeof(int4), hipMemcpyHostToDevice));
+        GRACE_TRY_HIP(hipMemsetAsync(pp.idx + words, 0, PLAN_IDX_PAD * sizeof(uint32_t), stream));
+        GRACE_TRY_HIP(hipMemsetAsync(pp.hdr + hdrs, 0, PLAN_HDR_PAD * sizeof(uint32_t), stream));
+        pp.key.subtiles = sub != 0;
+        GRACE_TRY_HIP(hipMemsetAsync(pp.ctl, 0, sizeof(PlanCtl), stream));
+        GRACE_TRY_HIP(hipMemsetD32Async(reinterpret_cast<hipDeviceptr_t>(&pp.ctl->usable), 1, 1, stream));
+        GRACE_TRY_HIP(hipMemcpyAsync(&pp.ctl->sig[0], ts.scene.ctl->sig, 16, hipMemcpyDeviceToDevice, stream));
+        GRACE_TRY_HIP(hipMemcpyAsync(&pp.ctl->sig[2], ts.rays.ctl->sig, 16, hipMemcpyDeviceToDevice, stream));
+        GRACE_TRY(launch_record(key.fast, sub != 0, a, PlanRef{ pp.idx, pp.hdr, pp.spans, pp.counts, pp.ctl, 1 }, stream));
+        pp.valid = true;
+        pp.dead = false;
+        return GRACE_OK;
+    }
     return GRACE_OK;
 }
 
 grace_status plan_record(const TraceState& ts, const TraceArgs& a, hipStream_t stream)
 {
     const PacketPlan& pp = ts.plan;
-    return launch_record(pp.key.fast, a, PlanRef{ pp.idx, pp.hdr, pp.spans, pp.counts, pp.ctl, 0 }, stream);
-}
-
-grace_status launch_planned(const int mode, const bool fast, const int grid, const TraceArgs& a, hipStream_t stream)
-{
+    return launch_record(pp.key.fast, pp.key.subtiles, a, PlanRef{ pp.idx, pp.hdr, pp.spans, pp.counts, pp.ctl, 0 }, stream);
+}
+
+grace_status launch_planned(const int mode, const bool fast, const bool subtiles, const int grid, const TraceArgs& a, hipStream_t stream)
+{
+    if (subtiles) {
+        if (mode != MODE_CUMULATIVE || !fast)
+            return set_error(GRACE_INVALID_ARGUMENT, __FILE__, __LINE__, "no sub-tile planned kernel for this mode");
+        trace_kernel<MODE_CUMULATIVE, true, true, false, true, true><<<grid, TRACE_BLOCK, 0, stream>>>(a);
+        GRACE_CHECK_LAUNCH();
+        return GRACE_OK;
+    }
     auto go = [&](auto mode_tag) {
         constexpr int MODE = decltype(mode_tag)::value;
         if (fast) trace_kernel<MODE, true, true, false, true><<<grid, TRACE_BLOCK, 0, stream>>>(a);
diff --git a/grace-devel_amd/csrc/trace_prepass.hip b/grace-devel_amd/csrc/trace_prepass.hip
--- a/grace-devel_amd/csrc/trace_prepass.hip
+++ b/grace-devel_amd/csrc/trace_prepass.hip
@@ -71,6 +71,7 @@
             b1 = make_float2(ir, ir * ir);
             b50 = make_float2(ir * float(N_TABLE - 1), fminf(ir * ir, 3.4028234664e38f));
         }
+        if (i == n) a.w = INFINITY;
         if (i < n + 4) {
             A[i] = a;
             if (B1) B1[i] = b1;
diff --git a/grace-devel_amd/csrc/trace_state.hpp b/grace-devel_amd/csrc/trace_state.hpp
--- a/grace-devel_amd/csrc/trace_state.hpp
+++ b/grace-devel_amd/csrc/trace_state.hpp
@@ -201,8 +201,13 @@
     unsigned long long stats[6];
     unsigned long long loops;
     uint32_t largest_loop, pad;
+    unsigned long long sub_steps, sub_slots;
 };
 constexpr int PLAN_FORMAT = 3;
+constexpr int PLAN_FORMAT_SUBTILE = 4;
+constexpr int PLAN_SUB_ROUND_STEPS = 16;
+constexpr int PLAN_SUB_MIN_PACKETS = 1024;
+constexpr double PLAN_SUB_MAX_RATIO = 0.82;
 __host__ __device__ inline uint32_t plan_header(const int n_surv, const int bits)
 {
     return uint32_t(n_surv) | (uint32_t(bits) << 8);
@@ -213,6 +218,7 @@
 
 struct PlanKey {
     int format = PLAN_FORMAT;
+    bool subtiles = false;
     bool fast = false;
     int group_shift = 0, width = 0;
     bool reorder = false;
@@ -220,7 +226,7 @@
     unsigned long long scene_gen = 0, rays_gen = 0;
     bool operator==(const PlanKey& o) const
     {
-        return format == o.format && fast == o.fast && group_shift == o.group_shift && width == o.width && reorder == o.reorder
+        return format == o.format && subtiles == o.subtiles && fast == o.fast && group_shift == o.group_shift && width == o.width && reorder == o.reorder
             && n_rays == o.n_rays && n_prims == o.n_prims && scene_gen == o.scene_gen && rays_gen == o.rays_gen;
     }
 };
@@ -229,6 +235,7 @@
     bool valid = false;
     bool dead = false;
     PlanKey key;
+    int asked = 0;
     uint32_t* idx = nullptr;
     uint32_t* hdr = nullptr;
     int4* spans = nullptr;
@@ -292,7 +299,8 @@
     double* custom_table = nullptr;
     double custom_host[N_TABLE] = {};
     bool plan_on = true;
-    size_t plan_budget = size_t(512) << 20;
+    size_t plan_budget = size_t(2) << 30;
+    int plan_subtiles = -1;
     Scene scene;
     RayOrder rays;
     HitsCache hits;
@@ -361,8 +369,8 @@
                                     const PlanGate* gate = nullptr, int* plan_split_dev = nullptr);
 
 grace_status plan_release(TraceState& ts);
-grace_status plan_fill(TraceState& ts, const PlanKey& key, const TraceArgs& a, hipStream_t stream);
+grace_status plan_fill(TraceState& ts, const PlanKey& key, int request, const TraceArgs& a, hipStream_t stream);
 grace_status plan_record(const TraceState& ts, const TraceArgs& a, hipStream_t stream);
-grace_status launch_planned(int mode, bool fast, int grid, const TraceArgs& a, hipStream_t stream);
-
-}
+grace_status launch_planned(int mode, bool fast, bool subtiles, int grid, const TraceArgs& a, hipStream_t stream);
+
+}
diff --git a/grace-devel_amd/grace_hip/__init__.py b/grace-devel_amd/grace_hip/__init__.py
--- a/grace-devel_amd/grace_hip/__init__.py
+++ b/grace-devel_amd/grace_hip/__init__.py
@@ -369,6 +369,16 @@
     v = (C.c_ulonglong * 2)()
     _check(_lib.grace_trace_plan_loops(v))
     return int(v[0]), int(v[1])
+
+
+def set_plan_subtiles(mode):
+    _check(_lib.grace_trace_set_plan_subtiles(C.c_int(int(mode))))
+
+
+def plan_subtiles():
+    used, steps, slots = C.c_int(0), C.c_ulonglong(0), C.c_ulonglong(0)
+    _check(_lib.grace_trace_plan_subtiles(C.byref(used), C.byref(steps), C.byref(slots)))
+    return used.value, int(steps.value), int(slots.value)
 
 
 def set_lattice_split(k):
diff --git a/include/grace_hip.h b/include/grace_hip.h
--- a/include/grace_hip.h
+++ b/include/grace_hip.h
@@ -242,6 +242,8 @@
 grace_status grace_trace_last_plan_used(int* h_used);
 grace_status grace_trace_plan_stats(unsigned long long* h_stats );
 grace_status grace_trace_plan_loops(unsigned long long* h_loops );
+grace_status grace_trace_set_plan_subtiles(int mode);
+grace_status grace_trace_plan_subtiles(int* h_used, unsigned long long* h_steps, unsigned long long* h_slots);
 
 grace_status grace_trace_status(grace_stream stream);
 
diff --git a/profiles/recipes/perf_subtiles.py b/profiles/recipes/perf_subtiles.py
--- /dev/null
+++ b/profiles/recipes/perf_subtiles.py
@@ -0,0 +1,54 @@
+import sys, os, statistics
+ROOT = os.path.dirname(os.path.dirname(os.path.dirname(os.path.abspath(__file__))))
+sys.path.insert(0, os.path.join(ROOT, "grace-devel_amd")); sys.path.insert(0, ROOT)
+import numpy as np
+import torch
+import grace_hip as gh
+from bench import make_particles
+dev = torch.device("cuda:0")
+n = 10_000_000
+s0 = make_particles(n, dev)
+gh.enable_kernel_timing(True)
+gh.set_plan_budget(12 << 30)
+
+
+def median_ms(call, reps=30):
+    for _ in range(5): call()
+    v = []
+    for _ in range(reps):
+        call(); v.append(gh.last_kernel_ms())
+    return statistics.median(v)
+
+
+def on_against_off(rays, s, tree, label):
+    out = torch.empty(len(rays), dtype=torch.float32, device=dev)
+    call = lambda: gh.trace_cumulative_sph(rays, s, tree, out)
+    row, bits = [], {}
+    for rep in range(2):
+        for mode in (0, 1):
+            gh.set_plan_subtiles(mode)
+            row.append("sub=%d %.4f" % (mode, median_ms(call)))
+            bits[mode] = out.cpu().numpy().view(np.uint32).copy()
+            if rep == 0:
+                used, steps, slots = gh.plan_subtiles()
+                surv = gh.plan_stats().survivors
+                row.append("[sub-tiles %d, %d survivors, steps / survivors %.4f, real words %.4f, %d bytes]"
+                           % (used, surv, steps / max(surv, 1), slots / max(4 * steps, 1), gh.plan_bytes()))
+    print("%s: %s  same bits: %s" % (label, "  ".join(row), np.array_equal(bits[0], bits[1])), flush=True)
+
+
+for scale in (1.0, 1.5, 2.0, 3.0, 4.0):
+    s = s0.clone()
+    s[:, 3] *= scale
+    lo, hi = gh.min_max_vec4(s); lo[3] = hi[3] = 0.0
+    tree = gh.Tree(n, 32, device=dev)
+    gh.build_tree(s, tree, lo[:3], hi[:3])
+    rays, _ = gh.orthogonal_rays_z(1024, lo, hi, device=dev)
+    if scale == 1.0:
+        for packets in (16384, 8192, 4096, 2048, 1024):
+            on_against_off(rays[: packets * 64].contiguous(), s, tree, "%d packets" % packets)
+    else:
+        packets = 4096 if scale <= 2.0 else 2048
+        on_against_off(rays[: packets * 64].contiguous(), s, tree, "h x %.1f, %d packets" % (scale, packets))
+    gh.set_plan_subtiles(0)
+    del tree
diff --git a/profiles/recipes/subtile_model.py b/profiles/recipes/subtile_model.py
--- /dev/null
+++ b/profiles/recipes/subtile_model.py
@@ -0,0 +1,60 @@
+import math
+import sys
+import numpy as np
+
+h_scale = float(sys.argv[1]) if len(sys.argv) > 1 else 1.0
+rng = np.random.default_rng(42)
+n = 10_000_000
+P = rng.random((n, 3), dtype=np.float32)
+h = h_scale * (3 * 48 / (4 * math.pi * n)) ** (1 / 3)
+
+
+def spread(v):
+    v = v.astype(np.uint64) & 0x3ff
+    v = (v | (v << 16)) & 0x030000FF
+    v = (v | (v << 8)) & 0x0300F00F
+    v = (v | (v << 4)) & 0x030C30C3
+    v = (v | (v << 2)) & 0x09249249
+    return v
+
+
+q = np.minimum((P * 1024).astype(np.int64), 1023)
+key = (spread(q[:, 0]) << 2) | (spread(q[:, 1]) << 1) | spread(q[:, 2])
+P = P[np.argsort(key, kind="stable")]
+pix = 1.0 / 1024
+
+
+def dist2_rect(x, y, x0, x1, y0, y1):
+    dx = x - np.clip(x, x0, x1)
+    dy = y - np.clip(y, y0, y1)
+    return dx * dx + dy * dy
+
+
+survivors = quadrant_steps = half_x_steps = half_y_steps = hits = 0
+tiles = rng.integers(8, 120, size=(40, 2))
+for tx, ty in tiles:
+    x0, y0 = (tx * 8 + 0.5) * pix, (ty * 8 + 0.5) * pix
+    near = (np.abs(P[:, 0] - (x0 + 3.5 * pix)) < 3.5 * pix + h) & (np.abs(P[:, 1] - (y0 + 3.5 * pix)) < 3.5 * pix + h)
+    idx = np.nonzero(near)[0]
+    x, y = P[idx, 0], P[idx, 1]
+    keep = dist2_rect(x, y, x0, x0 + 7 * pix, y0, y0 + 7 * pix) < h * h
+    idx, x, y = idx[keep], x[keep], y[keep]
+    cls = (idx >> 10) & 7
+    ox, oy = x0 + pix * np.arange(8), y0 + pix * np.arange(8)
+    hits += ((x[:, None, None] - ox[None, :, None]) ** 2 + (y[:, None, None] - oy[None, None, :]) ** 2 < h * h).sum()
+    quad = np.zeros((len(idx), 4), bool)
+    for qi in range(2):
+        for qj in range(2):
+            quad[:, qi * 2 + qj] = dist2_rect(x, y, x0 + 4 * qi * pix, x0 + (4 * qi + 3) * pix,
+                                              y0 + 4 * qj * pix, y0 + (4 * qj + 3) * pix) < h * h
+    lower_x, upper_x = quad[:, 0] | quad[:, 1], quad[:, 2] | quad[:, 3]
+    lower_y, upper_y = quad[:, 0] | quad[:, 2], quad[:, 1] | quad[:, 3]
+    for c in range(8):
+        mc = cls == c
+        survivors += mc.sum()
+        quadrant_steps += quad[mc].sum(axis=0).max()
+        half_x_steps += max(lower_x[mc].sum(), upper_x[mc].sum())
+        half_y_steps += max(lower_y[mc].sum(), upper_y[mc].sum())
+print("h = %.2f pixels: %.0f survivors per packet, fill %.3f" % (h / pix, survivors / len(tiles), hits / (survivors * 64)))
+print("steps kept: 4 x 4 quadrants %.3f, halves split in x %.3f, in y %.3f"
+      % (quadrant_steps / survivors, half_x_steps / survivors, half_y_steps / survivors))
diff --git a/profiles/recipes/subtile_read_ubench.hip b/profiles/recipes/subtile_read_ubench.hip
--- /dev/null
+++ b/profiles/recipes/subtile_read_ubench.hip
@@ -0,0 +1,137 @@
+#include <hip/hip_runtime.h>
+#include <cstdio>
+#include <cstring>
+#include <vector>
+#define CK(x) do { hipError_t e_ = (x); if (e_ != hipSuccess) { printf("HIP error %s line %d\n", hipGetErrorString(e_), __LINE__); return 1; } } while (0)
+
+typedef float f32x4 __attribute__((ext_vector_type(4)));
+
+constexpr int TILE = 132;
+constexpr int STEPS = TILE / 4;
+
+template <bool SUB>
+__global__ __launch_bounds__(256) void lds_kernel(float* out, int iters)
+{
+    __shared__ __align__(16) float4 tile[4][TILE];
+    const int wv = threadIdx.x >> 6, lane = threadIdx.x & 63;
+    for (int i = threadIdx.x; i < 4 * TILE * 4; i += 256) (&tile[0][0].x)[i] = float(i & 7);
+    __syncthreads();
+    const unsigned base = unsigned(reinterpret_cast<size_t>(&tile[wv][0])) + (SUB ? 16u * unsigned(lane >> 4) : 0u);
+    for (int i = 0; i < iters; ++i) {
+        const unsigned addr = base + (SUB ? unsigned(i % 28) * 64u : unsigned(i & 63) * 16u);
+        f32x4 p0, p1, p2, p3;
+        if (SUB) {
+            asm volatile("ds_read_b128 %0, %1" : "=v"(p0) : "v"(addr));
+            asm volatile("ds_read_b128 %0, %1 offset:64" : "=v"(p1) : "v"(addr));
+            asm volatile("ds_read_b128 %0, %1 offset:128" : "=v"(p2) : "v"(addr));
+            asm volatile("ds_read_b128 %0, %1 offset:192" : "=v"(p3) : "v"(addr));
+        } else {
+            asm volatile("ds_read_b128 %0, %1" : "=v"(p0) : "v"(addr));
+            asm volatile("ds_read_b128 %0, %1 offset:16" : "=v"(p1) : "v"(addr));
+            asm volatile("ds_read_b128 %0, %1 offset:32" : "=v"(p2) : "v"(addr));
+            asm volatile("ds_read_b128 %0, %1 offset:48" : "=v"(p3) : "v"(addr));
+        }
+        asm volatile("s_waitcnt lgkmcnt(0)" ::: "memory");
+        asm volatile("" :: "v"(p0), "v"(p1), "v"(p2), "v"(p3));
+    }
+    out[blockIdx.x * 256 + threadIdx.x] = float(lane);
+}
+
+template <bool SUB>
+__global__ __launch_bounds__(256, 8) void loop_kernel(float* out, int rounds, int n)
+{
+    __shared__ __align__(16) float4 tile[4][TILE];
+    __shared__ float2 s_lutf[256];
+    const int wv = threadIdx.x >> 6, lane = threadIdx.x & 63;
+    for (int i = threadIdx.x; i < 4 * TILE; i += 256) {
+        const int j = i % TILE;
+        tile[i / TILE][j] = make_float4(3.5f + 0.37f * float(j % 29) - 5.f, 3.5f + 0.53f * float(j % 23) - 6.f,
+                                        50.f / (10.f + 0.1f * float(j % 7)), 0.01f - 1e-5f * float(j % 11));
+    }
+    {
+        const float x = float(threadIdx.x) / 50.f, y0 = threadIdx.x < 50 ? (1.f - x) * (1.f - x) : 0.f;
+        const float x1 = float(threadIdx.x + 1) / 50.f, y1 = threadIdx.x + 1 < 50 ? (1.f - x1) * (1.f - x1) : 0.f;
+        const float dy = y1 - y0;
+        s_lutf[threadIdx.x] = threadIdx.x < 50 ? make_float2(y0 - float(threadIdx.x) * dy, dy) : make_float2(0.f, 0.f);
+    }
+    __syncthreads();
+    const float o1 = float(lane & 7), o2 = float(lane >> 3);
+    float sum = 0.f;
+    constexpr int S = SUB ? 4 : 1;
+    const float4* const tile4 = &tile[wv][0] + (SUB ? lane >> 4 : 0);
+    for (int r = 0; r < rounds; ++r) {
+        int left = n;
+        const float4* t4 = tile4 + S * (r & 1);
+        float4 c0, c1, c2;
+        auto proc = [&](const float4 c) {
+            const float q1 = c.x - o1, q2 = c.y - o2;
+            const float b = __builtin_amdgcn_sqrtf(__builtin_fmaf(q1, q1, q2 * q2)) * c.z;
+            const float2 y = s_lutf[static_cast<int>(b)];
+            sum = __builtin_fmaf(__builtin_fmaf(y.y, b, y.x), c.w, sum);
+        };
+        c0 = t4[0]; __builtin_amdgcn_sched_barrier(0);
+        c1 = t4[S]; __builtin_amdgcn_sched_barrier(0);
+        for (;;) {
+            c2 = t4[2 * S]; __builtin_amdgcn_sched_barrier(0);
+            proc(c0);
+            if (--left == 0) break;
+            c0 = t4[3 * S]; __builtin_amdgcn_sched_barrier(0);
+            proc(c1);
+            if (--left == 0) break;
+            c1 = t4[4 * S]; __builtin_amdgcn_sched_barrier(0);
+            proc(c2);
+            if (--left == 0) break;
+            t4 += 3 * S;
+        }
+    }
+    out[blockIdx.x * 256 + threadIdx.x] = sum;
+}
+
+template <typename F>
+static float time_ms(F launch)
+{
+    hipEvent_t e0, e1;
+    bool ok = hipEventCreate(&e0) == hipSuccess;
+    ok = hipEventCreate(&e1) == hipSuccess && ok;
+    launch();
+    ok = hipDeviceSynchronize() == hipSuccess && ok;
+    float best = 1e30f;
+    for (int rep = 0; rep < 3 && ok; ++rep) {
+        ok = hipEventRecord(e0) == hipSuccess && ok;
+        launch();
+        ok = hipEventRecord(e1) == hipSuccess && ok;
+        ok = hipEventSynchronize(e1) == hipSuccess && ok;
+        float ms = 0.f;
+        ok = hipEventElapsedTime(&ms, e0, e1) == hipSuccess && ok;
+        best = ms < best ? ms : best;
+    }
+    ok = hipGetLastError() == hipSuccess && ok;
+    (void)hipEventDestroy(e0); (void)hipEventDestroy(e1);
+    return ok ? best : -1.f;
+}
+#define TIMED(t) do { if ((t) < 0.f) { printf("HIP error while timing, line %d\n", __LINE__); return 1; } } while (0)
+
+int main()
+{
+    float* out;
+    const int blocks = 256 * 8;
+    const size_t n_out = size_t(blocks) * 256;
+    CK(hipMalloc(&out, n_out * sizeof(float)));
+    const int li = 16000;
+    const double per_cu = 32.0 * li * 4;
+    const float lu = time_ms([&] { lds_kernel<false><<<blocks, 256>>>(out, li); });
+    const float ls = time_ms([&] { lds_kernel<true><<<blocks, 256>>>(out, li); });
+    TIMED(lu); TIMED(ls);
+    printf("b. record read, ns per wave-read per CU (cycles at 2.4 GHz): uniform ds_read_b128 %.3f (%.2f) | sub-tile ds_read_b128 %.3f (%.2f) | ratio %.3f\n",
+           lu * 1e6 / per_cu, lu * 1e6 / per_cu * 2.4, ls * 1e6 / per_cu, ls * 1e6 / per_cu * 2.4, ls / lu);
+    const int rounds = 400, n = 30;
+    const float cu = time_ms([&] { loop_kernel<false><<<blocks, 256>>>(out, rounds, n); });
+    const float cs = time_ms([&] { loop_kernel<true><<<blocks, 256>>>(out, rounds, n); });
+    TIMED(cu); TIMED(cs);
+    const double steps_per_simd = 8.0 * rounds * n;
+    printf("c. survivor loop, %d rounds of %d steps: uniform form %.3f ms (%.2f ns per step per SIMD) | sub-tile form %.3f ms (%.2f ns) | sub-tile / uniform %.3f\n",
+           rounds, n, cu, cu * 1e6 / steps_per_simd, cs, cs * 1e6 / steps_per_simd, cs / cu);
+    CK(hipGetLastError());
+    CK(hipFree(out));
+    return 0;
+}
```
